# sabarim/STEm-Seg

Measured on AMD Instinct MI355X. Metric: clips/sec (T=8, 480p) embed+cluster, higher is better.
Workload: dtype f16x3: fp32 emulated from 2 fp16 terms per operand (22-bit operand significands; fp32 has 24), power-of-two operand scaling, 3 fp16 MFMA products per fp32 product, fp32 accumulate; |activation| >= 2.6e5 -> non-finite, flagged on the device, clip re-run in bf16x6

## Files before the change

stem-seg_amd/csrc/bottleneck_fused.hip:

```cpp
#include "common.h"
#include "split_operand.h"

namespace stemseg {

typedef float f32x16 __attribute__((ext_vector_type(16)));
typedef _Float16 f16x8 __attribute__((ext_vector_type(8)));
typedef unsigned int u32x4 __attribute__((ext_vector_type(4)));

struct FusedTailParams {
    const unsigned int* x16;
    const char* w3;
    const float* b3;
    const float* res;
    float* y;
    const char* w1;
    const float* b1;
    float* z;
    int64_t z_cs, z_ts, z_ys;
    int dec_H, dec_W;
    int V;
};

constexpr SplitLayout FT_WL = SplitLayout(1, STEMSEG_PRECISION_F16X3);
static_assert(FT_WL.CK == 32 && FT_WL.G == 2 && FT_WL.NPL == 2, "the fused tail walks 32-channel chunks of two k-groups, two planes");

template <int MID_, int CT_, int P_>
struct FusedTailCfg {
    static constexpr int MID = MID_, CT = CT_, COUT = 4 * MID_;
    static constexpr int P = P_, NW = P_ / 32, NTHREADS = 64 * NW;
    static constexpr int NC3 = MID / 32;
    static constexpr int NCT = COUT / CT;
    static constexpr int MI3 = CT / 32, MI1 = MID / 32;
    static constexpr int NH = 2 * MI3;
    static constexpr int X_BYTES = 2 * 4 * P * 16;
    static constexpr int W3_BYTES = 8 * CT * 16;
    static constexpr int W1_HALF = 4 * MID * 16;
    static constexpr int LDS_BYTES = 2 * X_BYTES + 2 * W3_BYTES + 2 * W1_HALF;
    static constexpr int NQ = P / 64;
    static constexpr int X_PIECES = X_BYTES / 1024, W3_PIECES = W3_BYTES / 1024, W1_PIECES = W1_HALF / 1024;
    static_assert(NC3 == FT_WL.chunks(MID) && W3_BYTES == FT_WL.slab_bytes(CT, 32) && W1_HALF * FT_WL.G == FT_WL.slab_bytes(MID, 32), "tile byte sizes follow the packed-weight layout");
    static_assert(P % 64 == 0 && MID % 32 == 0 && CT % 32 == 0 && COUT % CT == 0, "tile shapes");
    static_assert(LDS_BYTES <= (P <= 128 ? 80 : 160) * 1024, "LDS: two 128-position workgroups, or one 256-position workgroup, per CU");
    static_assert(W3_BYTES % 1024 == 0 && W1_HALF % 1024 == 0 && X_PIECES % NW == 0, "whole DMA pieces");
    static_assert(MI1 * 16 + MI3 * 16 <= 176, "accumulators must leave room for fragments at 256 registers");
};

template <class C>
__global__ __launch_bounds__(C::NTHREADS, 2) void fused_tail_kernel(const FusedTailParams p) {
#pragma clang fp contract(off)
    __shared__ __attribute__((aligned(1024))) char smem[C::LDS_BYTES];
    char* const xbuf = smem;
    char* const w3buf = smem + 2 * C::X_BYTES;
    char* const w1buf = smem + 2 * C::X_BYTES + 2 * C::W3_BYTES;

    const int tid = threadIdx.x, lane = tid & 63;
    const int wave = __builtin_amdgcn_readfirstlane(tid >> 6);
    const int half = lane >> 5, l31 = lane & 31;
    const int pos0 = blockIdx.x * C::P;
    const int pos = pos0 + wave * 32 + l31;
    const bool pos_ok = pos < p.V;
    const int pos_c = min(pos, p.V - 1);
    const int64_t V = p.V;
    const unsigned int lane_off = (unsigned int)(((int64_t)(4 * half) * V + pos_c) * 4);
    auto opaque = [](unsigned int v) __attribute__((always_inline)) { asm volatile("" : "+v"(v)); return v; };

    typedef const __attribute__((address_space(1))) void* gptr_t;
    typedef __attribute__((address_space(3))) void* lptr_t;
    const float* inv3 = reinterpret_cast<const float*>(p.w3 + FT_WL.inv_offset(C::COUT, C::MID));
    const float* inv1 = reinterpret_cast<const float*>(p.w1 + FT_WL.inv_offset(C::MID, C::COUT));

    const int xpos = min(pos0 + lane, p.V - 1);
    auto dma_x = [&](const int c, const int buf) __attribute__((always_inline)) {
#pragma unroll
        for (int k = 0; k < C::X_PIECES / C::NW; ++k) {
            const int idx = wave * (C::X_PIECES / C::NW) + k, q = idx % C::NQ, o = (idx / C::NQ) & 3, pl = idx / (4 * C::NQ);
            const unsigned int xp = (unsigned int)min((int)opaque((unsigned int)xpos) + q * 64, p.V - 1);
            const char* src = reinterpret_cast<const char*>(p.x16) + ((int64_t)(pl * (C::MID / 8) + 4 * c + o)) * V * 16 + (size_t)(xp * 16u);
            __builtin_amdgcn_global_load_lds((gptr_t)src, (lptr_t)(xbuf + buf * C::X_BYTES + ((pl * 4 + o) * C::P + q * 64) * 16), 16, 0, 0);
        }
    };
    auto dma_w3 = [&](const int j, const int c, const int buf) __attribute__((always_inline)) {
        constexpr int PER_ROW = C::CT * 16 / 1024;
#pragma unroll
        for (int k = 0; k < (C::W3_PIECES + C::NW - 1) / C::NW; ++k) {
            const int idx = wave + k * C::NW;
            if (idx < C::W3_PIECES) {
                const int row = idx / PER_ROW, part = idx % PER_ROW;
                const char* src = p.w3 + ((int64_t)c * 8 + row) * (C::COUT * 16) + (int64_t)j * (C::CT * 16) + part * 1024 + (size_t)(opaque((unsigned int)lane) * 16u);
                __builtin_amdgcn_global_load_lds((gptr_t)src, (lptr_t)(w3buf + buf * C::W3_BYTES + idx * 1024), 16, 0, 0);
            }
        }
    };
    auto dma_w1 = [&](const int j, const int h, const int buf) __attribute__((always_inline)) {
#pragma unroll
        for (int k = 0; k < (C::W1_PIECES + C::NW - 1) / C::NW; ++k) {
            const int idx = wave + k * C::NW;
            if (idx < C::W1_PIECES) {
                const char* src = p.w1 + ((int64_t)j * C::NH + h) * C::W1_HALF + (int64_t)idx * 1024 + (size_t)(opaque((unsigned int)lane) * 16u);
                __builtin_amdgcn_global_load_lds((gptr_t)src, (lptr_t)(w1buf + buf * C::W1_HALF + idx * 1024), 16, 0, 0);
            }
        }
    };
    auto dma_tab = [&](const int j, const int buf) __attribute__((always_inline)) {
        static_assert(2 * (C::CT / 4) <= 64 && 2 * C::CT * 4 <= C::W3_BYTES, "the table is one DMA piece");
        if (wave == 0 && lane < 2 * (C::CT / 4)) {
            const unsigned int l = opaque((unsigned int)lane);
            const float* src = (l < C::CT / 4 ? inv3 : p.b3 - C::CT) + (int64_t)j * C::CT + (size_t)(l * 4u);
            __builtin_amdgcn_global_load_lds((gptr_t)src, (lptr_t)(w3buf + buf * C::W3_BYTES), 16, 0, 0);
        }
    };
    auto dma_tail_tab = [&]() __attribute__((always_inline)) {
        constexpr int PIECES = (2 * C::MID + 255) / 256;
        if (wave < PIECES) {
            const unsigned int f0 = (unsigned int)wave * 256u + opaque((unsigned int)lane) * 4u;
            if (f0 < 2u * C::MID) {
                const float* src = (f0 < (unsigned int)C::MID ? inv1 : p.b1 - C::MID) + (size_t)f0;
                __builtin_amdgcn_global_load_lds((gptr_t)src, (lptr_t)(xbuf + wave * 1024), 16, 0, 0);
            }
        }
    };
    auto stage_sync = [&]() __attribute__((always_inline)) {
        __builtin_amdgcn_s_waitcnt(0x0f70);
        __syncthreads();
    };
    auto load_identity = [&](const int co_first, float (&rres)[16]) __attribute__((always_inline)) {
#pragma unroll
        for (int r = 0; r < 16; ++r)
            rres[r] = *reinterpret_cast<const float*>(reinterpret_cast<const char*>(p.res + (int64_t)(co_first + (r & 3) + 8 * (r >> 2)) * V) + (size_t)lane_off);
    };

    f32x16 acc1[C::MI1];
#pragma unroll
    for (int m = 0; m < C::MI1; ++m)
#pragma unroll
        for (int r = 0; r < 16; ++r) acc1[m][r] = 0.f;

    const f16x8 k2048 = {(_Float16)(1.0f / F16X3_LO_SCALE), (_Float16)(1.0f / F16X3_LO_SCALE), (_Float16)(1.0f / F16X3_LO_SCALE), (_Float16)(1.0f / F16X3_LO_SCALE),
                         (_Float16)(1.0f / F16X3_LO_SCALE), (_Float16)(1.0f / F16X3_LO_SCALE), (_Float16)(1.0f / F16X3_LO_SCALE), (_Float16)(1.0f / F16X3_LO_SCALE)};

    auto mma3 = [&](f32x16& acc, const f16x8 a_hi, const f16x8 a_lo, const f16x8 b_hi, const f16x8 b_lo) __attribute__((always_inline)) {
        const f16x8 a_his = a_hi * k2048;
        acc = __builtin_amdgcn_mfma_f32_32x32x16_f16(a_lo, b_hi, acc, 0, 0, 0);
        acc = __builtin_amdgcn_mfma_f32_32x32x16_f16(a_his, b_lo, acc, 0, 0, 0);
        acc = __builtin_amdgcn_mfma_f32_32x32x16_f16(a_hi, b_hi, acc, 0, 0, 0);
    };

    dma_x(0, 0);
    dma_w3(0, 0, 0);
    stage_sync();
    int sb = 0;
#pragma unroll 1
    for (int j = 0; j < C::NCT; ++j) {
        f32x16 acc3[C::MI3];
#pragma unroll
        for (int m = 0; m < C::MI3; ++m)
#pragma unroll
            for (int r = 0; r < 16; ++r) acc3[m][r] = 0.f;
        const int co_j = j * C::CT;
        float rres[16];
#pragma unroll 1
        for (int c = 0; c < C::NC3; ++c) {
            if (c + 1 < C::NC3) { dma_x(c + 1, sb ^ 1); dma_w3(j, c + 1, sb ^ 1); }
            else { dma_w1(j, 0, 0); dma_tab(j, sb ^ 1); load_identity(co_j, rres); }
            const char* xb = xbuf + sb * C::X_BYTES + (half * C::P + wave * 32 + l31) * 16;
            const char* wb = w3buf + sb * C::W3_BYTES + (half * C::CT + l31) * 16;
            constexpr int NS = 2 * C::MI3;
            f16x8 b_hi[2], b_lo[2], a_hi[2], a_lo[2];
            auto ld_b = [&](const int g, const int k) __attribute__((always_inline)) {
                b_hi[k] = *reinterpret_cast<const f16x8*>(xb + ((0 * 4 + 2 * g) * C::P) * 16);
                b_lo[k] = *reinterpret_cast<const f16x8*>(xb + ((1 * 4 + 2 * g) * C::P) * 16);
            };
            auto ld_a = [&](const int st, const int k) __attribute__((always_inline)) {
                const int g = st / C::MI3, m = st % C::MI3;
                a_hi[k] = *reinterpret_cast<const f16x8*>(wb + (((g * 2 + 0) * 2) * C::CT + m * 32) * 16);
                a_lo[k] = *reinterpret_cast<const f16x8*>(wb + (((g * 2 + 1) * 2) * C::CT + m * 32) * 16);
            };
            ld_b(0, 0);
            ld_b(1, 1);
            ld_a(0, 0);
#pragma unroll
            for (int st = 0; st < NS; ++st) {
                if (st + 1 < NS) ld_a(st + 1, (st + 1) & 1);
                __builtin_amdgcn_sched_barrier(0);
                mma3(acc3[st % C::MI3], a_hi[st & 1], a_lo[st & 1], b_hi[st / C::MI3], b_lo[st / C::MI3]);
                __builtin_amdgcn_sched_barrier(0);
            }
            stage_sync();
            sb ^= 1;
        }
        f16x8 b_hi[2], b_lo[2];
#pragma unroll
        for (int h = 0; h < C::NH; ++h) {
            const int m = h >> 1, g = h & 1;
            if (g == 0) {
                const int co_m = co_j + m * 32;
                unsigned int hw[8], lw[8];
                const float* tab = reinterpret_cast<const float*>(w3buf + sb * C::W3_BYTES);
                __builtin_amdgcn_sched_barrier(0);
#pragma unroll
                for (int q = 0; q < 4; ++q) {
                    const int co4 = co_m + 8 * q + 4 * half;
                    const float4 sc = *reinterpret_cast<const float4*>(tab + (co4 - co_j));
                    const float4 bv = *reinterpret_cast<const float4*>(tab + C::CT + (co4 - co_j));
                    float v0 = __fmul_rn(acc3[m][4 * q + 0], sc.x), v1 = __fmul_rn(acc3[m][4 * q + 1], sc.y), v2 = __fmul_rn(acc3[m][4 * q + 2], sc.z),
                          v3 = __fmul_rn(acc3[m][4 * q + 3], sc.w);
                    v0 = relu_keep_nan(__fadd_rn(__fadd_rn(v0, bv.x), rres[4 * q + 0]));
                    v1 = relu_keep_nan(__fadd_rn(__fadd_rn(v1, bv.y), rres[4 * q + 1]));
                    v2 = relu_keep_nan(__fadd_rn(__fadd_rn(v2, bv.z), rres[4 * q + 2]));
                    v3 = relu_keep_nan(__fadd_rn(__fadd_rn(v3, bv.w), rres[4 * q + 3]));
                    if (pos_ok) {
                        char* yo = reinterpret_cast<char*>(p.y + (int64_t)(co_m + 8 * q) * V);
                        *reinterpret_cast<float*>(yo + (size_t)lane_off) = v0;
                        *reinterpret_cast<float*>(yo + V * 4 + (size_t)lane_off) = v1;
                        *reinterpret_cast<float*>(yo + V * 8 + (size_t)lane_off) = v2;
                        *reinterpret_cast<float*>(yo + V * 12 + (size_t)lane_off) = v3;
                    }
                    split_pair_f16(v0, v1, hw[2 * q], lw[2 * q]);
                    split_pair_f16(v2, v3, hw[2 * q + 1], lw[2 * q + 1]);
                }
                __builtin_amdgcn_sched_barrier(0);
#pragma unroll
                for (int gg = 0; gg < 2; ++gg) {
                    unsigned int xh[2], yh[2], xl[2], yl[2];
#pragma unroll
                    for (int i = 0; i < 2; ++i) {
                        auto sh = __builtin_amdgcn_permlane32_swap(hw[4 * gg + i], hw[4 * gg + 2 + i], false, false);
                        xh[i] = sh[0]; yh[i] = sh[1];
                        auto sl = __builtin_amdgcn_permlane32_swap(lw[4 * gg + i], lw[4 * gg + 2 + i], false, false);
                        xl[i] = sl[0]; yl[i] = sl[1];
                    }
                    const u32x4 bh = {xh[0], xh[1], yh[0], yh[1]}, bl = {xl[0], xl[1], yl[0], yl[1]};
                    b_hi[gg] = __builtin_bit_cast(f16x8, bh);
                    b_lo[gg] = __builtin_bit_cast(f16x8, bl);
                }
            } else if (m + 1 < C::MI3) {
                load_identity(co_j + (m + 1) * 32, rres);
            }
            __builtin_amdgcn_sched_barrier(0);
            if (h + 1 < C::NH) dma_w1(j, h + 1, (h + 1) & 1);
            else if (j + 1 < C::NCT) { dma_x(0, sb); dma_w3(j + 1, 0, sb); }
            else dma_tail_tab();
            const char* w1b = w1buf + (h & 1) * C::W1_HALF + (half * C::MID + l31) * 16;
            f16x8 a_hi[2], a_lo[2];
            auto ld_a1 = [&](const int m1, const int k) __attribute__((always_inline)) {
                a_hi[k] = *reinterpret_cast<const f16x8*>(w1b + ((0 * 2) * C::MID + m1 * 32) * 16);
                a_lo[k] = *reinterpret_cast<const f16x8*>(w1b + ((1 * 2) * C::MID + m1 * 32) * 16);
            };
            ld_a1(0, 0);
#pragma unroll
            for (int m1 = 0; m1 < C::MI1; ++m1) {
                if (m1 + 1 < C::MI1) ld_a1(m1 + 1, (m1 + 1) & 1);
                __builtin_amdgcn_sched_barrier(0);
                mma3(acc1[m1], a_hi[m1 & 1], a_lo[m1 & 1], b_hi[g], b_lo[g]);
                __builtin_amdgcn_sched_barrier(0);
            }
            stage_sync();
        }
    }
    if (pos_ok) {
        const int hwp = p.dec_H * p.dec_W;
        const int t2 = pos / hwp, r2 = pos - t2 * hwp, y2 = r2 / p.dec_W, x2 = r2 - y2 * p.dec_W;
        const unsigned int z_off = (unsigned int)(((int64_t)(4 * half) * p.z_cs + (int64_t)t2 * p.z_ts + (int64_t)y2 * p.z_ys + x2) * 4);
#pragma unroll
        for (int m1 = 0; m1 < C::MI1; ++m1)
#pragma unroll
            for (int q = 0; q < 4; ++q) {
                const int co4 = m1 * 32 + 8 * q + 4 * half;
                const float4 sc = *reinterpret_cast<const float4*>(reinterpret_cast<const float*>(xbuf) + co4);
                const float4 bv = *reinterpret_cast<const float4*>(reinterpret_cast<const float*>(xbuf) + C::MID + co4);
                char* zo = reinterpret_cast<char*>(p.z + (int64_t)(m1 * 32 + 8 * q) * p.z_cs);
                *reinterpret_cast<float*>(zo + (size_t)z_off) = relu_keep_nan(__fadd_rn(__fmul_rn(acc1[m1][4 * q + 0], sc.x), bv.x));
                *reinterpret_cast<float*>(zo + p.z_cs * 4 + (size_t)z_off) = relu_keep_nan(__fadd_rn(__fmul_rn(acc1[m1][4 * q + 1], sc.y), bv.y));
                *reinterpret_cast<float*>(zo + p.z_cs * 8 + (size_t)z_off) = relu_keep_nan(__fadd_rn(__fmul_rn(acc1[m1][4 * q + 2], sc.z), bv.z));
                *reinterpret_cast<float*>(zo + p.z_cs * 12 + (size_t)z_off) = relu_keep_nan(__fadd_rn(__fmul_rn(acc1[m1][4 * q + 3], sc.w), bv.w));
            }
    }
}


typedef float f32x4 __attribute__((ext_vector_type(4)));

template <int MID_>
struct FusedTail16Cfg {
    static constexpr int MID = MID_, COUT = 4 * MID_, CT = 128;
    static constexpr int NW = 8, NTHREADS = 512, P = 16 * NW;
    static constexpr int NC3 = MID / 32, NCT = COUT / CT;
    static constexpr int NT3 = CT / 16, NT1 = MID / 16;
    static constexpr int SC = 2;
    static constexpr int NS = NC3 / SC, NU = CT / 32;
    static constexpr int W3_CHUNK = 8 * CT * 16;
    static constexpr int W3_BYTES = SC * W3_CHUNK;
    static constexpr int W1_BYTES = 8 * MID * 16;
    static constexpr int TAB_BYTES = 2 * CT * 4;
    static constexpr int LDS_BYTES = 2 * W3_BYTES + 2 * W1_BYTES + 2 * TAB_BYTES;
    static_assert(NC3 % SC == 0 && W3_BYTES % (1024 * NW) == 0 && W1_BYTES % (1024 * NW) == 0 && TAB_BYTES == 1024, "whole DMA pieces per wave");
    static_assert(W3_CHUNK == FT_WL.slab_bytes(CT, FT_WL.CK) && W1_BYTES == FT_WL.slab_bytes(MID, FT_WL.CK), "tile byte sizes follow the packed-weight layout");
    static_assert(LDS_BYTES <= 160 * 1024 && 2 * MID * 4 <= W3_BYTES, "LDS");
};

template <class C>
__global__ __launch_bounds__(C::NTHREADS, 2) void fused_tail16_kernel(const FusedTailParams p) {
#pragma clang fp contract(off)
    __shared__ __attribute__((aligned(1024))) char smem[C::LDS_BYTES];
    char* const w3buf = smem;
    char* const w1buf = smem + 2 * C::W3_BYTES;
    char* const tabbuf = smem + 2 * C::W3_BYTES + 2 * C::W1_BYTES;

    const int tid = threadIdx.x, lane = tid & 63;
    const int wave = __builtin_amdgcn_readfirstlane(tid >> 6);
    const int n = lane & 15, kb = lane >> 4;
    const int pos = blockIdx.x * C::P + wave * 16 + n;
    const bool pos_ok = pos < p.V;
    const int pos_c = min(pos, p.V - 1);
    const int64_t V = p.V;
    const unsigned int lane_off = (unsigned int)(((int64_t)(4 * kb) * V + pos_c) * 4);
    auto opaque = [](unsigned int v) __attribute__((always_inline)) { asm volatile("" : "+v"(v)); return v; };
    typedef const __attribute__((address_space(1))) void* gptr_t;
    typedef __attribute__((address_space(3))) void* lptr_t;
    const float* inv3 = reinterpret_cast<const float*>(p.w3 + FT_WL.inv_offset(C::COUT, C::MID));
    const float* inv1 = reinterpret_cast<const float*>(p.w1 + FT_WL.inv_offset(C::MID, C::COUT));

    auto dma_w3 = [&](const int j, const int st, const int buf) __attribute__((always_inline)) {
        constexpr int PER_ROW = C::CT * 16 / 1024, PER_CHUNK = C::W3_CHUNK / 1024;
#pragma unroll
        for (int k = 0; k < C::W3_BYTES / 1024 / C::NW; ++k) {
            const int idx = wave + k * C::NW, sc = idx / PER_CHUNK, r = idx % PER_CHUNK, row = r / PER_ROW, part = r % PER_ROW;
            const char* src = p.w3 + ((int64_t)(st * C::SC + sc) * 8 + row) * (C::COUT * 16) + (int64_t)j * (C::CT * 16) + part * 1024 + (size_t)(opaque((unsigned int)lane) * 16u);
            __builtin_amdgcn_global_load_lds((gptr_t)src, (lptr_t)(w3buf + buf * C::W3_BYTES + idx * 1024), 16, 0, 0);
        }
    };
    auto dma_w1 = [&](const int cc, const int buf) __attribute__((always_inline)) {
#pragma unroll
        for (int k = 0; k < C::W1_BYTES / 1024 / C::NW; ++k) {
            const int idx = wave + k * C::NW;
            const char* src = p.w1 + (int64_t)cc * C::W1_BYTES + (int64_t)idx * 1024 + (size_t)(opaque((unsigned int)lane) * 16u);
            __builtin_amdgcn_global_load_lds((gptr_t)src, (lptr_t)(w1buf + buf * C::W1_BYTES + idx * 1024), 16, 0, 0);
        }
    };
    auto dma_tab = [&](const int j) __attribute__((always_inline)) {
        if (wave == 0) {
            const unsigned int l = opaque((unsigned int)lane);
            const float* src = (l < 32 ? inv3 : p.b3 - C::CT) + (int64_t)j * C::CT + (size_t)(l * 4u);
            __builtin_amdgcn_global_load_lds((gptr_t)src, (lptr_t)(tabbuf + (j & 1) * C::TAB_BYTES), 16, 0, 0);
        }
    };
    auto dma_tail_tab = [&]() __attribute__((always_inline)) {
        constexpr int PIECES = (2 * C::MID + 255) / 256;
        if (wave < PIECES) {
            const unsigned int f0 = (unsigned int)wave * 256u + opaque((unsigned int)lane) * 4u;
            if (f0 < 2u * C::MID) {
                const float* src = (f0 < (unsigned int)C::MID ? inv1 : p.b1 - C::MID) + (size_t)f0;
                __builtin_amdgcn_global_load_lds((gptr_t)src, (lptr_t)(w3buf + wave * 1024), 16, 0, 0);
            }
        }
    };
    auto stage_sync = [&]() __attribute__((always_inline)) {
        __builtin_amdgcn_s_waitcnt(0x0f70);
        __syncthreads();
    };
    auto load_identity = [&](const int co_first, float (&rres)[8]) __attribute__((always_inline)) {
#pragma unroll
        for (int i = 0; i < 8; ++i)
            rres[i] = *reinterpret_cast<const float*>(reinterpret_cast<const char*>(p.res + (int64_t)(co_first + 16 * (i >> 2) + (i & 3)) * V) + (size_t)lane_off);
    };
    const f16x8 k2048 = {(_Float16)(1.0f / F16X3_LO_SCALE), (_Float16)(1.0f / F16X3_LO_SCALE), (_Float16)(1.0f / F16X3_LO_SCALE), (_Float16)(1.0f / F16X3_LO_SCALE),
                         (_Float16)(1.0f / F16X3_LO_SCALE), (_Float16)(1.0f / F16X3_LO_SCALE), (_Float16)(1.0f / F16X3_LO_SCALE), (_Float16)(1.0f / F16X3_LO_SCALE)};
    auto mma3x2 = [&](f32x4& c0, f32x4& c1, const f16x8 a0_hi, const f16x8 a0_lo, const f16x8 a1_hi, const f16x8 a1_lo, const f16x8 b_hi, const f16x8 b_lo)
        __attribute__((always_inline)) {
        const f16x8 a0_his = a0_hi * k2048, a1_his = a1_hi * k2048;
        c0 = __builtin_amdgcn_mfma_f32_16x16x32_f16(a0_lo, b_hi, c0, 0, 0, 0);
        c1 = __builtin_amdgcn_mfma_f32_16x16x32_f16(a1_lo, b_hi, c1, 0, 0, 0);
        c0 = __builtin_amdgcn_mfma_f32_16x16x32_f16(a0_his, b_lo, c0, 0, 0, 0);
        c1 = __builtin_amdgcn_mfma_f32_16x16x32_f16(a1_his, b_lo, c1, 0, 0, 0);
        c0 = __builtin_amdgcn_mfma_f32_16x16x32_f16(a0_hi, b_hi, c0, 0, 0, 0);
        c1 = __builtin_amdgcn_mfma_f32_16x16x32_f16(a1_hi, b_hi, c1, 0, 0, 0);
    };

    dma_w3(0, 0, 0);
    f16x8 xh[C::NC3], xl[C::NC3];
    {
        const char* xs = reinterpret_cast<const char*>(p.x16) + (size_t)((unsigned int)pos_c * 16u);
#pragma unroll
        for (int s = 0; s < C::NC3; ++s) {
            xh[s] = *reinterpret_cast<const f16x8*>(xs + ((int64_t)(4 * s + kb)) * V * 16);
            xl[s] = *reinterpret_cast<const f16x8*>(xs + ((int64_t)(C::MID / 8 + 4 * s + kb)) * V * 16);
        }
    }
    f32x4 acc1[C::NT1];
#pragma unroll
    for (int m = 0; m < C::NT1; ++m) acc1[m] = f32x4{0.f, 0.f, 0.f, 0.f};
    stage_sync();
    int sb = 0, eb = 0;
#pragma unroll 1
    for (int j = 0; j < C::NCT; ++j) {
        f32x4 acc3[C::NT3];
#pragma unroll
        for (int t = 0; t < C::NT3; ++t) acc3[t] = f32x4{0.f, 0.f, 0.f, 0.f};
        const int co_j = j * C::CT;
        float rres[8];
#pragma unroll
        for (int st = 0; st < C::NS; ++st) {
            if (st + 1 < C::NS) dma_w3(j, st + 1, sb ^ 1);
            else { dma_w1(j * C::NU, eb); dma_tab(j); load_identity(co_j, rres); }
            const char* wb = w3buf + sb * C::W3_BYTES + (((kb >> 1) * 2 * 2 + (kb & 1)) * C::CT + n) * 16;
            constexpr int NSTEP = C::SC * C::NT3 / 2;
            f16x8 a_hi[2][2], a_lo[2][2];
            auto ld_a = [&](const int i, const int k) __attribute__((always_inline)) {
                const int sc = (2 * i) / C::NT3, t = (2 * i) % C::NT3;
#pragma unroll
                for (int e = 0; e < 2; ++e) {
                    a_hi[k][e] = *reinterpret_cast<const f16x8*>(wb + sc * C::W3_CHUNK + (0 * 2 * C::CT + (t + e) * 16) * 16);
                    a_lo[k][e] = *reinterpret_cast<const f16x8*>(wb + sc * C::W3_CHUNK + (1 * 2 * C::CT + (t + e) * 16) * 16);
                }
            };
            ld_a(0, 0);
#pragma unroll
            for (int i = 0; i < NSTEP; ++i) {
                if (i + 1 < NSTEP) ld_a(i + 1, (i + 1) & 1);
                __builtin_amdgcn_sched_barrier(0);
                const int t = (2 * i) % C::NT3, ch = st * C::SC + (2 * i) / C::NT3;
                mma3x2(acc3[t], acc3[t + 1], a_hi[i & 1][0], a_lo[i & 1][0], a_hi[i & 1][1], a_lo[i & 1][1], xh[ch], xl[ch]);
                __builtin_amdgcn_sched_barrier(0);
            }
            stage_sync();
            sb ^= 1;
        }
        const float* tab = reinterpret_cast<const float*>(tabbuf + (j & 1) * C::TAB_BYTES);
#pragma unroll
        for (int u = 0; u < C::NU; ++u) {
            unsigned int hw[4], lw[4];
            __builtin_amdgcn_sched_barrier(0);
#pragma unroll
            for (int tt = 0; tt < 2; ++tt) {
                const int t = 2 * u + tt, co4 = 16 * t + 4 * kb;
                const float4 sc = *reinterpret_cast<const float4*>(tab + co4);
                const float4 bv = *reinterpret_cast<const float4*>(tab + C::CT + co4);
                float v0 = __fmul_rn(acc3[t][0], sc.x), v1 = __fmul_rn(acc3[t][1], sc.y), v2 = __fmul_rn(acc3[t][2], sc.z), v3 = __fmul_rn(acc3[t][3], sc.w);
                v0 = relu_keep_nan(__fadd_rn(__fadd_rn(v0, bv.x), rres[4 * tt + 0]));
                v1 = relu_keep_nan(__fadd_rn(__fadd_rn(v1, bv.y), rres[4 * tt + 1]));
                v2 = relu_keep_nan(__fadd_rn(__fadd_rn(v2, bv.z), rres[4 * tt + 2]));
                v3 = relu_keep_nan(__fadd_rn(__fadd_rn(v3, bv.w), rres[4 * tt + 3]));
                if (pos_ok) {
                    char* yo = reinterpret_cast<char*>(p.y + (int64_t)(co_j + 16 * t) * V);
                    *reinterpret_cast<float*>(yo + (size_t)lane_off) = v0;
                    *reinterpret_cast<float*>(yo + V * 4 + (size_t)lane_off) = v1;
                    *reinterpret_cast<float*>(yo + V * 8 + (size_t)lane_off) = v2;
                    *reinterpret_cast<float*>(yo + V * 12 + (size_t)lane_off) = v3;
                }
                split_pair_f16(v0, v1, hw[2 * tt], lw[2 * tt]);
                split_pair_f16(v2, v3, hw[2 * tt + 1], lw[2 * tt + 1]);
            }
            unsigned int bw[2][4];
#pragma unroll
            for (int pl = 0; pl < 2; ++pl)
#pragma unroll
                for (int i = 0; i < 2; ++i) {
                    const unsigned int t0 = pl ? lw[i] : hw[i], t1 = pl ? lw[2 + i] : hw[2 + i];
                    auto s32 = __builtin_amdgcn_permlane32_swap(t0, t1, false, false);
                    auto s16 = __builtin_amdgcn_permlane16_swap(s32[0], s32[1], false, false);
                    bw[pl][i] = s16[0];
                    bw[pl][2 + i] = s16[1];
                }
            const u32x4 bh = {bw[0][0], bw[0][1], bw[0][2], bw[0][3]}, bl = {bw[1][0], bw[1][1], bw[1][2], bw[1][3]};
            const f16x8 b_hi = __builtin_bit_cast(f16x8, bh), b_lo = __builtin_bit_cast(f16x8, bl);
            __builtin_amdgcn_sched_barrier(0);
            if (u + 1 < C::NU) { dma_w1(j * C::NU + u + 1, eb ^ 1); load_identity(co_j + 32 * (u + 1), rres); }
            else if (j + 1 < C::NCT) dma_w3(j + 1, 0, sb);
            else dma_tail_tab();
            __builtin_amdgcn_sched_barrier(0);
            const char* w1b = w1buf + eb * C::W1_BYTES + (((kb >> 1) * 2 * 2 + (kb & 1)) * C::MID + n) * 16;
            f16x8 a_hi[1][2], a_lo[1][2];
            auto ld_a1 = [&](const int i, const int k) __attribute__((always_inline)) {
#pragma unroll
                for (int e = 0; e < 2; ++e) {
                    a_hi[k][e] = *reinterpret_cast<const f16x8*>(w1b + (0 * 2 * C::MID + (2 * i + e) * 16) * 16);
                    a_lo[k][e] = *reinterpret_cast<const f16x8*>(w1b + (1 * 2 * C::MID + (2 * i + e) * 16) * 16);
                }
            };
#pragma unroll
            for (int i = 0; i < C::NT1 / 2; ++i) {
                ld_a1(i, 0);
                __builtin_amdgcn_sched_barrier(0);
                mma3x2(acc1[2 * i], acc1[2 * i + 1], a_hi[0][0], a_lo[0][0], a_hi[0][1], a_lo[0][1], b_hi, b_lo);
                __builtin_amdgcn_sched_barrier(0);
            }
            stage_sync();
            eb ^= 1;
        }
    }
    if (pos_ok) {
        const int hwp = p.dec_H * p.dec_W;
        const int t2 = pos / hwp, r2 = pos - t2 * hwp, y2 = r2 / p.dec_W, x2 = r2 - y2 * p.dec_W;
        const unsigned int z_off = (unsigned int)(((int64_t)(4 * kb) * p.z_cs + (int64_t)t2 * p.z_ts + (int64_t)y2 * p.z_ys + x2) * 4);
        const float* ttab = reinterpret_cast<const float*>(w3buf);
#pragma unroll
        for (int m1 = 0; m1 < C::NT1; ++m1) {
            const int co4 = m1 * 16 + 4 * kb;
            const float4 sc = *reinterpret_cast<const float4*>(ttab + co4);
            const float4 bv = *reinterpret_cast<const float4*>(ttab + C::MID + co4);
            char* zo = reinterpret_cast<char*>(p.z + (int64_t)(m1 * 16) * p.z_cs);
            *reinterpret_cast<float*>(zo + (size_t)z_off) = relu_keep_nan(__fadd_rn(__fmul_rn(acc1[m1][0], sc.x), bv.x));
            *reinterpret_cast<float*>(zo + p.z_cs * 4 + (size_t)z_off) = relu_keep_nan(__fadd_rn(__fmul_rn(acc1[m1][1], sc.y), bv.y));
            *reinterpret_cast<float*>(zo + p.z_cs * 8 + (size_t)z_off) = relu_keep_nan(__fadd_rn(__fmul_rn(acc1[m1][2], sc.z), bv.z));
            *reinterpret_cast<float*>(zo + p.z_cs * 12 + (size_t)z_off) = relu_keep_nan(__fadd_rn(__fmul_rn(acc1[m1][3], sc.w), bv.w));
        }
    }
}


typedef __amdgpu_buffer_rsrc_t ft_rsrc_t;
#define FT_VMCNT_(n) __builtin_amdgcn_s_waitcnt(((n) & 15) | (((n) >> 4) << 14) | 0x0F70)
#define FT_VMCNT(n) FT_VMCNT_(n)
#define FT_SGB(mask, n) __builtin_amdgcn_sched_group_barrier(mask, n, 0)

template <int MID_, int CT_>
struct FusedTailR1Cfg {
    static constexpr int MID = MID_, CT = CT_, COUT = 4 * MID_;
    static constexpr int NW = 4, NTHREADS = 64 * NW, P = 32 * NW;
    static constexpr int NC3 = MID / 32, NG = MID / 16, NCT = COUT / CT;
    static constexpr int MI3 = CT / 32, MI1 = MID / 32;
    static constexpr int SC = 2;
    static constexpr int NS = NC3 / SC, NU = CT / 32;
    static constexpr int NX3 = SC * 2 * (MI3 / 2), NX1 = 2 * (MI1 / 2);
    static constexpr int W3_CHUNK = 8 * CT * 16, W3_BYTES = SC * W3_CHUNK;
    static constexpr int W1_BYTES = 8 * MID * 16;
    static_assert(W3_CHUNK == FT_WL.slab_bytes(CT, FT_WL.CK) && W1_BYTES == FT_WL.slab_bytes(MID, FT_WL.CK), "tile byte sizes follow the packed-weight layout");
    static constexpr int TAB_BYTES = 1024;
    static constexpr int LDS_BYTES = 2 * W3_BYTES + 2 * W1_BYTES + 2 * TAB_BYTES;
    static constexpr int W3_PIECES = W3_BYTES / 1024 / NW, W1_PIECES = W1_BYTES / 1024 / NW;
    static constexpr int SL = 8 / NX1, S0 = NX1 / 4, M_PPS = 8 / S0;
    static_assert(NC3 % SC == 0 && MI3 % 2 == 0 && MI1 % 2 == 0 && W3_BYTES % (1024 * NW) == 0 && W1_BYTES % (1024 * NW) == 0 && 2 * CT * 4 <= TAB_BYTES, "whole DMA pieces per wave");
    static_assert(LDS_BYTES <= 160 * 1024 && 2 * MID * 4 <= W3_BYTES && (NX1 == 8 || NX1 == 4) && NX3 == 8 && MI3 == 4 && NS >= 2 && NU >= 2 && NU % 2 == 0, "LDS / slice placement / identity buffer parity");
    static_assert(W3_PIECES == 8 && W1_PIECES <= 8, "the pieces of a stage are requested in its first steps");
    static_assert(NG * 8 + MI1 * 16 <= 256, "the conv3 input and conv1's accumulators are the AGPR half of the register file");
};

template <class C>
__global__ __launch_bounds__(C::NTHREADS, 1) void fused_tail_r1_kernel(const FusedTailParams p) {
#pragma clang fp contract(off)
    __shared__ __attribute__((aligned(1024))) char smem[C::LDS_BYTES];
    char* const w3buf = smem;
    char* const w1buf = smem + 2 * C::W3_BYTES;
    char* const tabbuf = smem + 2 * C::W3_BYTES + 2 * C::W1_BYTES;

    const int tid = threadIdx.x, lane = tid & 63;
    const int wave = __builtin_amdgcn_readfirstlane(tid >> 6);
    const int half = lane >> 5, l31 = lane & 31;
    const int pos = blockIdx.x * C::P + wave * 32 + l31;
    const bool pos_ok = pos < p.V;
    const int pos_c = min(pos, p.V - 1);
    const int64_t V = p.V;
    const unsigned int V4 = (unsigned int)p.V * 4u;
    const unsigned int lane_ld = (unsigned int)(4 * half) * V4 + (unsigned int)pos_c * 4u;
    const unsigned int lane_st = pos_ok ? lane_ld : 0xFFFFFF00u;
    const unsigned int tile_bytes = (unsigned int)C::CT * V4;
    typedef __attribute__((address_space(3))) void* lptr_t;
    const float* inv3 = reinterpret_cast<const float*>(p.w3 + FT_WL.inv_offset(C::COUT, C::MID));
    const float* inv1 = reinterpret_cast<const float*>(p.w1 + FT_WL.inv_offset(C::MID, C::COUT));

    const unsigned int lane16 = (unsigned int)lane * 16u;
    const unsigned int lds_w3 = (unsigned int)(uintptr_t)(lptr_t)w3buf, lds_w1 = (unsigned int)(uintptr_t)(lptr_t)w1buf;
    auto dma_piece = [&](const char* sbase, const unsigned int lds_addr) __attribute__((always_inline)) {
        asm volatile("s_mov_b32 m0, %0\n\ts_nop 0\n\tglobal_load_lds_dwordx4 %1, %2" : : "s"(lds_addr), "v"(lane16), "s"(sbase) : "memory");
    };
    auto dma_w3 = [&](const int j, const int st, const int buf, const int k) __attribute__((always_inline)) {
        constexpr int PER_ROW = C::CT * 16 / 1024, PER_CHUNK = C::W3_CHUNK / 1024;
        const int idx = wave + k * C::NW, sc = idx / PER_CHUNK, r = idx % PER_CHUNK, row = r / PER_ROW, part = r % PER_ROW;
        dma_piece(p.w3 + ((int64_t)(st * C::SC + sc) * 8 + row) * (C::COUT * 16) + (int64_t)j * (C::CT * 16) + part * 1024, lds_w3 + buf * C::W3_BYTES + idx * 1024);
    };
    auto dma_w1 = [&](const int cc, const int buf, const int k) __attribute__((always_inline)) {
        const int idx = wave + k * C::NW;
        dma_piece(p.w1 + (int64_t)cc * C::W1_BYTES + (int64_t)idx * 1024, lds_w1 + buf * C::W1_BYTES + idx * 1024);
    };
    float4 tabv = {0.f, 0.f, 0.f, 0.f};
    auto tab_fetch = [&](const int j) __attribute__((always_inline)) {
        if (wave == 0 && lane < 2 * (C::CT / 4))
            tabv = *reinterpret_cast<const float4*>((lane < C::CT / 4 ? inv3 : p.b3 - C::CT) + (int64_t)j * C::CT + lane * 4);
    };
    auto tab_store = [&](const int j) __attribute__((always_inline)) {
        if (wave == 0 && lane < 2 * (C::CT / 4)) *reinterpret_cast<float4*>(tabbuf + (j & 1) * C::TAB_BYTES + lane * 16) = tabv;
    };
    auto rsrc_of = [&](const float* base, const int jj) __attribute__((always_inline)) {
        return __builtin_amdgcn_make_buffer_rsrc(const_cast<float*>(base + (int64_t)jj * C::CT * V), 0, (int)tile_bytes, 0x00020000);
    };
    auto load_identity = [&](const int jj, const int u, float (&rr)[16]) __attribute__((always_inline)) {
        const ft_rsrc_t rs = rsrc_of(p.res, jj);
#pragma unroll
        for (int r = 0; r < 16; ++r)
            rr[r] = __builtin_bit_cast(float, __builtin_amdgcn_raw_buffer_load_b32(rs, lane_ld, (unsigned int)(32 * u + (r & 3) + 8 * (r >> 2)) * V4, 0));
    };
    const f16x8 k2048 = {(_Float16)(1.0f / F16X3_LO_SCALE), (_Float16)(1.0f / F16X3_LO_SCALE), (_Float16)(1.0f / F16X3_LO_SCALE), (_Float16)(1.0f / F16X3_LO_SCALE),
                         (_Float16)(1.0f / F16X3_LO_SCALE), (_Float16)(1.0f / F16X3_LO_SCALE), (_Float16)(1.0f / F16X3_LO_SCALE), (_Float16)(1.0f / F16X3_LO_SCALE)};
    auto mma6 = [&](f32x16& c0, f32x16& c1, const f16x8 (&a_hi)[2], const f16x8 (&a_lo)[2], const f16x8 (&a_his)[2], const f16x8 b_hi, const f16x8 b_lo)
        __attribute__((always_inline)) {
        c0 = __builtin_amdgcn_mfma_f32_32x32x16_f16(a_lo[0], b_hi, c0, 0, 0, 0);
        c1 = __builtin_amdgcn_mfma_f32_32x32x16_f16(a_lo[1], b_hi, c1, 0, 0, 0);
        c0 = __builtin_amdgcn_mfma_f32_32x32x16_f16(a_his[0], b_lo, c0, 0, 0, 0);
        c1 = __builtin_amdgcn_mfma_f32_32x32x16_f16(a_his[1], b_lo, c1, 0, 0, 0);
        c0 = __builtin_amdgcn_mfma_f32_32x32x16_f16(a_hi[0], b_hi, c0, 0, 0, 0);
        c1 = __builtin_amdgcn_mfma_f32_32x32x16_f16(a_hi[1], b_hi, c1, 0, 0, 0);
    };

#pragma unroll
    for (int k = 0; k < C::W3_PIECES; ++k) dma_w3(0, 0, 0, k);
    float rres[2][16];
    load_identity(0, 0, rres[0]);
    load_identity(0, 1, rres[1]);
    f16x8 xh[C::NG], xl[C::NG];
    {
        const char* xs = reinterpret_cast<const char*>(p.x16) + (size_t)((unsigned int)pos_c * 16u);
#pragma unroll
        for (int G = 0; G < C::NG; ++G) {
            xh[G] = *reinterpret_cast<const f16x8*>(xs + ((int64_t)(2 * G + half)) * V * 16);
            xl[G] = *reinterpret_cast<const f16x8*>(xs + ((int64_t)(C::MID / 8 + 2 * G + half)) * V * 16);
        }
    }
    f32x16 acc1[C::MI1];
#pragma unroll
    for (int m = 0; m < C::MI1; ++m)
#pragma unroll
        for (int r = 0; r < 16; ++r) acc1[m][r] = 0.f;
    FT_VMCNT(0);
    __syncthreads();
    int sb = 0, eb = 0;
#pragma unroll 1
    for (int j = 0; j < C::NCT; ++j) {
        f32x16 acc3[C::MI3];
#pragma unroll
        for (int m = 0; m < C::MI3; ++m)
#pragma unroll
            for (int r = 0; r < 16; ++r) acc3[m][r] = 0.f;
        const float* tab = reinterpret_cast<const float*>(tabbuf + (j & 1) * C::TAB_BYTES) + 4 * half;
        const ft_rsrc_t ry = rsrc_of(p.y, j);
        unsigned int hw[8], lw[8];
        f16x8 b_hi[2][2], b_lo[2][2];
        auto e_slice = [&](const int u, const int q4) __attribute__((always_inline)) {
            const int c4 = 32 * u + 8 * q4;
            const float4 sc = *reinterpret_cast<const float4*>(tab + c4);
            const float4 bv = *reinterpret_cast<const float4*>(tab + C::CT + c4);
            float (&rr)[16] = rres[u & 1];
            float v0 = __fmul_rn(acc3[u][4 * q4 + 0], sc.x), v1 = __fmul_rn(acc3[u][4 * q4 + 1], sc.y), v2 = __fmul_rn(acc3[u][4 * q4 + 2], sc.z),
                  v3 = __fmul_rn(acc3[u][4 * q4 + 3], sc.w);
            v0 = relu_keep_nan(__fadd_rn(__fadd_rn(v0, bv.x), rr[4 * q4 + 0]));
            v1 = relu_keep_nan(__fadd_rn(__fadd_rn(v1, bv.y), rr[4 * q4 + 1]));
            v2 = relu_keep_nan(__fadd_rn(__fadd_rn(v2, bv.z), rr[4 * q4 + 2]));
            v3 = relu_keep_nan(__fadd_rn(__fadd_rn(v3, bv.w), rr[4 * q4 + 3]));
            __builtin_amdgcn_raw_buffer_store_b32(__builtin_bit_cast(unsigned int, v0), ry, lane_st, (unsigned int)(c4 + 0) * V4, 0);
            __builtin_amdgcn_raw_buffer_store_b32(__builtin_bit_cast(unsigned int, v1), ry, lane_st, (unsigned int)(c4 + 1) * V4, 0);
            __builtin_amdgcn_raw_buffer_store_b32(__builtin_bit_cast(unsigned int, v2), ry, lane_st, (unsigned int)(c4 + 2) * V4, 0);
            __builtin_amdgcn_raw_buffer_store_b32(__builtin_bit_cast(unsigned int, v3), ry, lane_st, (unsigned int)(c4 + 3) * V4, 0);
            split_pair_f16(v0, v1, hw[2 * q4], lw[2 * q4]);
            split_pair_f16(v2, v3, hw[2 * q4 + 1], lw[2 * q4 + 1]);
        };
        auto e_perm = [&](const int gg, f16x8& bh, f16x8& bl) __attribute__((always_inline)) {
            unsigned int xh_[2], yh_[2], xl_[2], yl_[2];
#pragma unroll
            for (int i = 0; i < 2; ++i) {
                auto sh = __builtin_amdgcn_permlane32_swap(hw[4 * gg + i], hw[4 * gg + 2 + i], false, false);
                xh_[i] = sh[0]; yh_[i] = sh[1];
                auto sl = __builtin_amdgcn_permlane32_swap(lw[4 * gg + i], lw[4 * gg + 2 + i], false, false);
                xl_[i] = sl[0]; yl_[i] = sl[1];
            }
            const u32x4 bh4 = {xh_[0], xh_[1], yh_[0], yh_[1]}, bl4 = {xl_[0], xl_[1], yl_[0], yl_[1]};
            bh = __builtin_bit_cast(f16x8, bh4);
            bl = __builtin_bit_cast(f16x8, bl4);
        };
#pragma unroll
        for (int st = 0; st < C::NS; ++st) {
            if (st + 2 == C::NS) tab_fetch(j);
            const char* wb = w3buf + sb * C::W3_BYTES + (half * C::CT + l31) * 16;
            f16x8 a_hi[3][2], a_lo[3][2], a_his[2][2];
            auto ld3 = [&](const int s, const int k) __attribute__((always_inline)) {
                const int mp = s / (2 * C::SC), sc = (s % (2 * C::SC)) / 2, g = s % 2;
#pragma unroll
                for (int e = 0; e < 2; ++e) {
                    a_hi[k][e] = *reinterpret_cast<const f16x8*>(wb + sc * C::W3_CHUNK + (((g * 2 + 0) * 2) * C::CT + (2 * mp + e) * 32) * 16);
                    a_lo[k][e] = *reinterpret_cast<const f16x8*>(wb + sc * C::W3_CHUNK + (((g * 2 + 1) * 2) * C::CT + (2 * mp + e) * 32) * 16);
                }
            };
            ld3(0, 0);
            ld3(1, 1);
            a_his[0][0] = a_hi[0][0] * k2048;
            a_his[0][1] = a_hi[0][1] * k2048;
#pragma unroll
            for (int s = 0; s < C::NX3; ++s) {
                __builtin_amdgcn_sched_barrier(0);
                if (s < 2) {
#pragma unroll
                    for (int k = 4 * s; k < 4 * s + 4; ++k) {
                        if (st + 1 < C::NS) dma_w3(j, st + 1, sb ^ 1, k);
                        else if (k < C::W1_PIECES) dma_w1(j * C::NU, eb, k);
                    }
                }
                if (s + 2 < C::NX3) ld3(s + 2, (s + 2) % 3);
                if (s + 1 < C::NX3) {
                    a_his[(s + 1) & 1][0] = a_hi[(s + 1) % 3][0] * k2048;
                    a_his[(s + 1) & 1][1] = a_hi[(s + 1) % 3][1] * k2048;
                }
                if (st + 1 == C::NS && s >= C::NX3 / 2) e_slice(0, s - C::NX3 / 2);
                const int mp = s / (2 * C::SC), sc = (s % (2 * C::SC)) / 2, g = s % 2, G = 2 * (st * C::SC + sc) + g;
                mma6(acc3[2 * mp], acc3[2 * mp + 1], a_hi[s % 3], a_lo[s % 3], a_his[s & 1], xh[G], xl[G]);
#pragma unroll
                for (int i = 0; i < 6; ++i) {
                    FT_SGB(0x008, 1); FT_SGB(0x100, 1);
                    if (st + 1 == C::NS && s >= C::NX3 / 2) { FT_SGB(0x002, 7); FT_SGB(0x040, 1); }
                    else FT_SGB(0x002, 2);
                }
            }
            __builtin_amdgcn_sched_barrier(0);
            if (st + 1 == C::NS) FT_VMCNT(16);
            else FT_VMCNT(0);
            if (st + 2 == C::NS) tab_store(j);
            __syncthreads();
            sb ^= 1;
        }
        e_perm(0, b_hi[0][0], b_lo[0][0]);
        e_perm(1, b_hi[0][1], b_lo[0][1]);
#pragma unroll
        for (int u = 0; u < C::NU; ++u) {
            const char* w1b = w1buf + eb * C::W1_BYTES + (half * C::MID + l31) * 16;
            f16x8 a_hi[3][2], a_lo[3][2], a_his[2][2];
            auto ld1 = [&](const int s, const int k) __attribute__((always_inline)) {
                const int g = s / (C::MI1 / 2), mp = s % (C::MI1 / 2);
#pragma unroll
                for (int e = 0; e < 2; ++e) {
                    a_hi[k][e] = *reinterpret_cast<const f16x8*>(w1b + (((g * 2 + 0) * 2) * C::MID + (2 * mp + e) * 32) * 16);
                    a_lo[k][e] = *reinterpret_cast<const f16x8*>(w1b + (((g * 2 + 1) * 2) * C::MID + (2 * mp + e) * 32) * 16);
                }
            };
            ld1(0, 0);
            ld1(1, 1);
            a_his[0][0] = a_hi[0][0] * k2048;
            a_his[0][1] = a_hi[0][1] * k2048;
#pragma unroll
            for (int s = 0; s < C::NX1; ++s) {
                __builtin_amdgcn_sched_barrier(0);
                if (s < C::S0) {
#pragma unroll
                    for (int k = C::M_PPS * s; k < C::M_PPS * s + C::M_PPS; ++k) {
                        if (u + 1 < C::NU) { if (k < C::W1_PIECES) dma_w1(j * C::NU + u + 1, eb ^ 1, k); }
                        else if (j + 1 < C::NCT) dma_w3(j + 1, 0, sb, k);
                    }
                }
                if (s == C::S0) load_identity(u + 2 < C::NU ? j : min(j + 1, C::NCT - 1), (u + 2) % C::NU, rres[u & 1]);
                if (s + 2 < C::NX1) ld1(s + 2, (s + 2) % 3);
                if (s + 1 < C::NX1) {
                    a_his[(s + 1) & 1][0] = a_hi[(s + 1) % 3][0] * k2048;
                    a_his[(s + 1) & 1][1] = a_hi[(s + 1) % 3][1] * k2048;
                }
                if (u + 1 < C::NU) {
                    constexpr int SE = C::S0 + 4 / C::SL;
                    if (s >= C::S0 && s < SE) {
#pragma unroll
                        for (int q = 0; q < C::SL; ++q) e_slice(u + 1, (s - C::S0) * C::SL + q);
                    }
                    if (C::SL == 1 ? s == SE : s == SE) e_perm(0, b_hi[(u + 1) & 1][0], b_lo[(u + 1) & 1][0]);
                    if (C::SL == 1 ? s == SE + 1 : s == SE) e_perm(1, b_hi[(u + 1) & 1][1], b_lo[(u + 1) & 1][1]);
                }
                const int g = s / (C::MI1 / 2), mp = s % (C::MI1 / 2);
                mma6(acc1[2 * mp], acc1[2 * mp + 1], a_hi[s % 3], a_lo[s % 3], a_his[s & 1], b_hi[u & 1][g], b_lo[u & 1][g]);
#pragma unroll
                for (int i = 0; i < 6; ++i) { FT_SGB(0x008, 1); FT_SGB(0x100, 1); FT_SGB(0x002, 7 * C::SL); FT_SGB(0x040, C::SL); FT_SGB(0x020, 3); }
            }
            __builtin_amdgcn_sched_barrier(0);
            if (u + 1 < C::NU) FT_VMCNT(32);
            else FT_VMCNT(16);
            __syncthreads();
            eb ^= 1;
        }
    }
    static_assert(C::MID / 4 <= 64, "one lane per four channels");
    if (wave < 2 && lane < C::MID / 4)
        *reinterpret_cast<float4*>(w3buf + wave * (C::MID * 4) + lane * 16) = *reinterpret_cast<const float4*>((wave == 0 ? inv1 : p.b1) + lane * 4);
    __syncthreads();
    if (pos_ok) {
        const int hwp = p.dec_H * p.dec_W;
        const int t2 = pos / hwp, r2 = pos - t2 * hwp, y2 = r2 / p.dec_W, x2 = r2 - y2 * p.dec_W;
        const unsigned int z_off = (unsigned int)(((int64_t)(4 * half) * p.z_cs + (int64_t)t2 * p.z_ts + (int64_t)y2 * p.z_ys + x2) * 4);
        const float* ttab = reinterpret_cast<const float*>(w3buf);
#pragma unroll
        for (int m1 = 0; m1 < C::MI1; ++m1)
#pragma unroll
            for (int q = 0; q < 4; ++q) {
                const int co4 = m1 * 32 + 8 * q + 4 * half;
                const float4 sc = *reinterpret_cast<const float4*>(ttab + co4);
                const float4 bv = *reinterpret_cast<const float4*>(ttab + C::MID + co4);
                char* zo = reinterpret_cast<char*>(p.z + (int64_t)(m1 * 32 + 8 * q) * p.z_cs);
                *reinterpret_cast<float*>(zo + (size_t)z_off) = relu_keep_nan(__fadd_rn(__fmul_rn(acc1[m1][4 * q + 0], sc.x), bv.x));
                *reinterpret_cast<float*>(zo + p.z_cs * 4 + (size_t)z_off) = relu_keep_nan(__fadd_rn(__fmul_rn(acc1[m1][4 * q + 1], sc.y), bv.y));
                *reinterpret_cast<float*>(zo + p.z_cs * 8 + (size_t)z_off) = relu_keep_nan(__fadd_rn(__fmul_rn(acc1[m1][4 * q + 2], sc.z), bv.z));
                *reinterpret_cast<float*>(zo + p.z_cs * 12 + (size_t)z_off) = relu_keep_nan(__fadd_rn(__fmul_rn(acc1[m1][4 * q + 3], sc.w), bv.w));
            }
    }
}

template <class C>
static int launch_fused_r1_cfg(const FusedTailParams& p, hipStream_t s) {
    const double flops = 2.0 * 2.0 * (double)C::MID * C::COUT * (double)p.V;
    void* ev = profile_begin(19, flops, s);
    hipLaunchKernelGGL(fused_tail_r1_kernel<C>, dim3((unsigned)ceil_div(p.V, C::P)), dim3(C::NTHREADS), 0, s, p);
    profile_end(ev, s);
    SS_LAUNCH_CHECK();
    return STEMSEG_OK;
}

template <class C>
static int launch_fused16_cfg(const FusedTailParams& p, hipStream_t s) {
    const double flops = 2.0 * 2.0 * (double)C::MID * C::COUT * (double)p.V;
    void* ev = profile_begin(19, flops, s);
    hipLaunchKernelGGL(fused_tail16_kernel<C>, dim3((unsigned)ceil_div(p.V, C::P)), dim3(C::NTHREADS), 0, s, p);
    profile_end(ev, s);
    SS_LAUNCH_CHECK();
    return STEMSEG_OK;
}

template <class C>
static int launch_fused_cfg(const FusedTailParams& p, hipStream_t s) {
    const double flops = 2.0 * 2.0 * (double)C::MID * C::COUT * (double)p.V;
    void* ev = profile_begin(19, flops, s);
    hipLaunchKernelGGL(fused_tail_kernel<C>, dim3((unsigned)ceil_div(p.V, C::P)), dim3(C::NTHREADS), 0, s, p);
    profile_end(ev, s);
    SS_LAUNCH_CHECK();
    return STEMSEG_OK;
}

bool fused_tail_supported(int mid) { return mid == 64 || mid == 128 || mid == 256; }

int launch_fused_tail(int mid, const unsigned int* x16, const float* w3, const float* b3, const float* res, float* y, const float* w1, const float* b1,
                      const StemsegVolume& z, int dec_H, int dec_W, int64_t V, int form, hipStream_t s) {
    SS_CHECK_ARG(x16 && w3 && b3 && res && y && w1 && b1 && z.ptr, "fused_tail: null pointer");
    SS_CHECK_ARG(fused_tail_supported(mid), "fused_tail: mid = %d (64, 128 or 256)", mid);
    SS_CHECK_ARG(V > 0 && V <= (1ll << 27) && z.c_stride <= (1ll << 27) && dec_H > 0 && dec_W > 0 && V % ((int64_t)dec_H * dec_W) == 0, "fused_tail: V = %lld positions of %d x %d planes",
                 (long long)V, dec_H, dec_W);
    SS_CHECK_ARG(z.C == mid, "fused_tail: consumer volume has %d channels, conv1 makes %d", z.C, mid);
    SS_CHECK_ARG(reinterpret_cast<uintptr_t>(x16) % 16 == 0 && reinterpret_cast<uintptr_t>(w3) % 16 == 0 && reinterpret_cast<uintptr_t>(w1) % 16 == 0 &&
                 reinterpret_cast<uintptr_t>(b3) % 16 == 0 && reinterpret_cast<uintptr_t>(b1) % 16 == 0, "fused_tail: 16-byte aligned operands");
    FusedTailParams p;
    p.x16 = x16; p.w3 = reinterpret_cast<const char*>(w3); p.b3 = b3; p.res = res; p.y = y;
    p.w1 = reinterpret_cast<const char*>(w1); p.b1 = b1;
    p.z = z.ptr; p.z_cs = z.c_stride; p.z_ts = z.t_stride; p.z_ys = z.y_stride; p.dec_H = dec_H; p.dec_W = dec_W;
    p.V = (int)V;
    if (mid == 256) {
        const bool r1_fits = (int64_t)128 * V * 4 < (1ll << 32) - (1 << 20);
        if (form != 1 && r1_fits) return launch_fused_r1_cfg<FusedTailR1Cfg<256, 128>>(p, s);
        return launch_fused16_cfg<FusedTail16Cfg<256>>(p, s);
    }
    if (mid == 128 && form != 1 && (int64_t)128 * V * 4 < (1ll << 32) - (1 << 20)) return launch_fused_r1_cfg<FusedTailR1Cfg<128, 128>>(p, s);
    if (mid == 128) return launch_fused_cfg<FusedTailCfg<128, 128, 128>>(p, s);
    return launch_fused_cfg<FusedTailCfg<64, 128, 128>>(p, s);
}

}
```

stem-seg_amd/csrc/common.h:

```cpp
#pragma once
#include <hip/hip_runtime.h>
#include <cstdarg>
#include <cstdint>
#include <cstdio>
#include <cstring>

#include "../../include/stemseg_hip.h"

#if defined(__HIP_DEVICE_COMPILE__) && defined(__AMDGCN_WAVEFRONT_SIZE) && __AMDGCN_WAVEFRONT_SIZE != 64
#error "libstemseg_hip is written for 64-lane wavefronts (gfx950): shuffles, ballots and MFMA layouts assume it"
#endif

namespace stemseg {

void set_error(const char* fmt, ...);

#define SS_CHECK_ARG(cond, ...)                                     \
    do {                                                            \
        if (!(cond)) {                                              \
            ::stemseg::set_error(__VA_ARGS__);                      \
            return STEMSEG_E_INVALID;                               \
        }                                                           \
    } while (0)

#define SS_HIP(call)                                                                            \
    do {                                                                                        \
        hipError_t e_ = (call);                                                                 \
        if (e_ != hipSuccess) {                                                                 \
            ::stemseg::set_error("%s failed: %s (%s:%d)", #call, hipGetErrorString(e_),         \
                                 __FILE__, __LINE__);                                           \
            return STEMSEG_E_HIP;                                                               \
        }                                                                                       \
    } while (0)

#define SS_LAUNCH_CHECK() SS_HIP(hipGetLastError())

static inline hipStream_t as_stream(void* s) { return reinterpret_cast<hipStream_t>(s); }
static inline int64_t ceil_div(int64_t a, int64_t b) { return (a + b - 1) / b; }
static inline int64_t round_up(int64_t a, int64_t b) { return ceil_div(a, b) * b; }

__device__ __forceinline__ float relu_keep_nan(float v) { return v < 0.f ? 0.f : v; }
__device__ __forceinline__ float max_keep_nan(float a, float b) { return (a > b || a != a) ? a : b; }

struct PaddedGeom {
    int64_t pitch, ts, cs, total, interior;
    PaddedGeom() = default;
    PaddedGeom(int C, int T, int H, int W) {
        pitch = round_up((int64_t)W + 2, 4);
        ts = (int64_t)(H + 2) * pitch;
        cs = (int64_t)(T + 2) * ts;
        total = (int64_t)C * cs + 64;
        interior = ts + pitch + 1;
    }
};

static inline StemsegVolume make_volume(float* ptr, int64_t cs, int64_t ts, int64_t ys, int C, int T, int H, int W,
                                        int64_t limit) {
    StemsegVolume v;
    v.ptr = ptr; v.c_stride = cs; v.t_stride = ts; v.y_stride = ys; v.C = C; v.T = T; v.H = H; v.W = W; v.limit = limit;
    return v;
}
static inline StemsegVolume dense_volume(float* ptr, int C, int T, int H, int W) {
    return make_volume(ptr, (int64_t)T * H * W, (int64_t)H * W, W, C, T, H, W, (int64_t)C * T * H * W);
}
static inline StemsegVolume padded_halo_view(float* base, int C, int T, int H, int W) {
    PaddedGeom g(C, T, H, W);
    return make_volume(base, g.cs, g.ts, g.pitch, C, T + 2, H + 2, W + 2, g.total);
}
static inline StemsegVolume padded_interior_view(float* base, int C, int T, int H, int W) {
    PaddedGeom g(C, T, H, W);
    return make_volume(base + g.interior, g.cs, g.ts, g.pitch, C, T, H, W, g.total - g.interior);
}

constexpr int WS_GUARD_FLOATS = 64;
constexpr uint32_t WS_CANARY = 0x7fc5ca7au;
constexpr int WS_MAX_GUARDS = 64;
struct GuardList {
    int n = 0;
    int64_t off[WS_MAX_GUARDS];
    bool full = false;
    void push(int64_t o) { if (n < WS_MAX_GUARDS) off[n++] = o; else full = true; }
};
int launch_canary_fill(float* ws, const GuardList& g, hipStream_t s);
int canary_check(const float* ws, const GuardList& g, int32_t* n_bad_host, int64_t* first_bad_host, hipStream_t s);

void* profile_begin(int tag, double work, hipStream_t s);
void profile_end(void* handle, hipStream_t s);

struct ConvEpilogue {
    int relu = 0;
    const float* res = nullptr;
    int64_t res_cs = 0, res_ts = 0, res_ys = 0;
    int dec_H = 0, dec_W = 0;
    int precision = 0;
    int frames = 0, plan_frames = 0;
    int64_t plan_scratch_floats = 0;
    double* gn_part = nullptr;
    int gn_cpg = 0, gn_cap = 0;
    int* gn_used = nullptr;
    int nb = 1;
    int64_t in_bs = 0, out_bs = 0, gn_bs = 0;
    unsigned int* p16_out = nullptr;
    int* p16_done = nullptr;
    int zero_t_halo = 0;
};
int launch_conv3d(const StemsegVolume& in, const float* packed_w, const float* bias, const StemsegVolume& out,
                  int kt, int kh, int kw, int tile_cfg, hipStream_t s, float* splitk_scratch = nullptr, int64_t splitk_scratch_floats = 0,
                  const ConvEpilogue* epi = nullptr);
int launch_grouped_conv(const StemsegVolume& in, const void* packed_w, const float* bias, const StemsegVolume& out, int groups, int stride,
                        int relu, int precision, hipStream_t s);
bool fused_tail_supported(int mid);
int launch_fused_tail(int mid, const unsigned int* x16, const float* w3, const float* b3, const float* res, float* y, const float* w1, const float* b1,
                      const StemsegVolume& z, int dec_H, int dec_W, int64_t V, int form, hipStream_t s);
int launch_gn_stats(const float* x, int C, int64_t S, int groups, float eps, float* stats, double* scratch, hipStream_t s);
constexpr int GN_SLOT_CAP = 32768;
static inline int64_t gn_scratch_doubles(int Cout, int groups) { return (int64_t)groups * GN_SLOT_CAP * 2 > (int64_t)groups * 128 ? (int64_t)groups * GN_SLOT_CAP * 2 : (int64_t)groups * 128; }
int launch_conv3d_gn(const StemsegVolume& in, const float* packed_w, const float* bias, const StemsegVolume& out, int kt, int kh, int kw,
                     int tile_cfg, hipStream_t s, float* splitk_scratch, int64_t splitk_scratch_floats, const ConvEpilogue* epi, int groups,
                     float eps, float* stats, double* gn_scratch, int64_t stats_bs = 0);
int launch_gn_identity_stats(float* stats, int groups, hipStream_t s);
struct ClipBatch {
    int nb = 1;
    int64_t in_bs = 0, out_bs = 0, stats_bs = 0;
};
int launch_gn_finalize_slots(const double* part, int groups, int cap, int used, double group_elems, float eps, float* stats, hipStream_t s,
                             int nb = 1, int64_t part_bs = 0, int64_t stats_bs = 0);
int launch_gn_relu_pool(const float* x, int C, int T, int H, int W, int groups, const float* stats, const float* gamma,
                        const float* beta, int pool, const StemsegVolume& out, hipStream_t s, const ClipBatch& cb = ClipBatch());
int launch_upsample(const float* in, int C, int T, int H, int W, int st, int sy, int sx, const StemsegVolume& out,
                    hipStream_t s, const ClipBatch& cb = ClipBatch());
int launch_copy_to_volume(const float* in, int layout, const StemsegVolume& out, hipStream_t s);
int launch_copy_strided(const float* in, int64_t in_c_stride, int64_t in_t_stride, const StemsegVolume& out, hipStream_t s);
struct HeadSpec {
    int n_out;
    int act[STEMSEG_MAX_EMB_DIMS * 2];
    int grid_axis[STEMSEG_MAX_EMB_DIMS * 2];
};
struct HeadsGN {
    const float* stats;
    const float* gamma;
    const float* beta;
    int cpg;
    int64_t stats_bs;
};
int launch_heads(const float* x, int Cin, int T, int H, int W, const float* w, const float* bias, const HeadSpec& hs,
                 const float* gt, const float* gy, const float* gx, float* out, hipStream_t s, const ClipBatch& cb = ClipBatch(),
                 const float* add = nullptr, int64_t add_bs = 0, const HeadsGN* gn = nullptr);
int launch_level_head(const float* x, int Cin, int64_t V, const float* w, int n_out, const float* add, float* out, hipStream_t s, int nb, int64_t x_bs,
                      int64_t add_bs, int64_t out_bs);

}
```

stem-seg_amd/csrc/encoder.hip:

```cpp
#include "common.h"
#include <algorithm>
#include <cstddef>

namespace stemseg {

struct Padded2D {
    int64_t pitch, ts, cs, total, interior;
    Padded2D() = default;
    Padded2D(int C, int T, int H, int W) {
        pitch = round_up((int64_t)W + 2, 4);
        ts = (int64_t)(H + 2) * pitch;
        cs = (int64_t)T * ts;
        total = (int64_t)C * cs + 64;
        interior = pitch + 1;
    }
};
static inline StemsegVolume halo2d_view(float* base, int C, int T, int H, int W) {
    Padded2D g(C, T, H, W);
    return make_volume(base, g.cs, g.ts, g.pitch, C, T, H + 2, W + 2, g.total);
}
static inline StemsegVolume interior2d_view(float* base, int C, int T, int H, int W) {
    Padded2D g(C, T, H, W);
    return make_volume(base + g.interior, g.cs, g.ts, g.pitch, C, T, H, W, g.total - g.interior);
}
static inline StemsegVolume flat_view(float* base, int C, int64_t V) { return make_volume(base, V, 0, 0, C, 1, 1, (int)V, (int64_t)C * V); }

constexpr int ST_ROWS = 8, ST_COLS = 64, ST_PR = 2 * ST_ROWS + 5, ST_PC = 2 * ST_COLS + 5;

constexpr int SM_PW = 68, SM_ROWS_IN = 2 * ST_ROWS + 6;
constexpr int SM_PLANE = 3 * SM_ROWS_IN * SM_PW;
constexpr int SM_KSTEPS = 3 * 7 * 4;
typedef float f32x16s __attribute__((ext_vector_type(16)));
__global__ __launch_bounds__(256, 2) void stem_conv7x7_mfma_kernel(const float* __restrict__ frames, const float* __restrict__ w_tap_major,
                                                                 const float* __restrict__ bias, float* __restrict__ out, int T, int H, int W) {
    __shared__ __attribute__((aligned(16))) float lds[2 * SM_PLANE + SM_KSTEPS * 2 * 64];
    float* const planes = lds;
    float* const wl = lds + 2 * SM_PLANE;
    const int Ho = H / 2, Wo = W / 2;
    const int tiles_x = (Wo + ST_COLS - 1) / ST_COLS, tiles_y = (Ho + ST_ROWS - 1) / ST_ROWS;
    int b = blockIdx.x;
    const int tx = b % tiles_x; b /= tiles_x;
    const int ty = b % tiles_y;
    const int t = b / tiles_y;
    const int oy0 = ty * ST_ROWS, ox0 = tx * ST_COLS;
    const int iy0 = 2 * oy0 - 3, ix0 = 2 * ox0 - 3;
    for (int i = threadIdx.x; i < SM_KSTEPS * 2 * 64; i += 256) {
        const int co = i & 63, half = (i >> 6) & 1, step = i >> 7;
        const int q = step & 3, cdy = step >> 2, dx = 2 * q + half;
        wl[i] = dx < 7 ? w_tap_major[(cdy * 7 + dx) * 64 + co] : 0.f;
    }
    for (int i = threadIdx.x; i < 2 * SM_PLANE; i += 256) {
        const int par = i / SM_PLANE, r = i - par * SM_PLANE;
        const int xi = r % SM_PW, yy = (r / SM_PW) % SM_ROWS_IN, c = r / (SM_PW * SM_ROWS_IN);
        const int iy = iy0 + yy, ix = ix0 + 2 * xi + par;
        float v = 0.f;
        if (yy < ST_PR && 2 * xi + par < ST_PC && iy >= 0 && iy < H && ix >= 0 && ix < W) v = frames[(((int64_t)t * 3 + c) * H + iy) * W + ix];
        planes[i] = v;
    }
    __syncthreads();
    const int lane = threadIdx.x & 63, wave = threadIdx.x >> 6, half = lane >> 5, l31 = lane & 31;
    f32x16s acc[2][4];
#pragma unroll
    for (int mi = 0; mi < 2; ++mi)
#pragma unroll
        for (int ni = 0; ni < 4; ++ni)
#pragma unroll
            for (int r = 0; r < 16; ++r) acc[mi][ni][r] = 0.f;
    const float* a_ptr = wl + half * 64 + l31;
    const float* b_ptr[4];
#pragma unroll
    for (int ni = 0; ni < 4; ++ni) b_ptr[ni] = planes + half * SM_PLANE + (2 * (2 * wave + (ni >> 1))) * SM_PW + (ni & 1) * 32 + l31;
    auto ld = [&](const int step, float (&a)[2], float (&bv)[4]) __attribute__((always_inline)) {
        const int q = step & 3, cdy = step >> 2, c = cdy / 7, dy = cdy - 7 * c;
        const int boff = (c * SM_ROWS_IN + dy) * SM_PW + q;
#pragma unroll
        for (int mi = 0; mi < 2; ++mi) a[mi] = a_ptr[step * 128 + mi * 32];
#pragma unroll
        for (int ni = 0; ni < 4; ++ni) bv[ni] = b_ptr[ni][boff];
    };
    auto mm = [&](const float (&a)[2], const float (&bv)[4]) __attribute__((always_inline)) {
#pragma unroll
        for (int mi = 0; mi < 2; ++mi)
#pragma unroll
            for (int ni = 0; ni < 4; ++ni) acc[mi][ni] = __builtin_amdgcn_mfma_f32_32x32x2f32(a[mi], bv[ni], acc[mi][ni], 0, 0, 0);
    };
    float a0[2], b0[4], a1[2], b1[4];
    ld(0, a0, b0);
#pragma unroll
    for (int i = 0; i < SM_KSTEPS; i += 2) {
        ld(i + 1, a1, b1);
        __builtin_amdgcn_sched_barrier(0);
        mm(a0, b0);
        __builtin_amdgcn_sched_barrier(0);
        if (i + 2 < SM_KSTEPS) ld(i + 2, a0, b0);
        __builtin_amdgcn_sched_barrier(0);
        mm(a1, b1);
        __builtin_amdgcn_sched_barrier(0);
    }
    const int64_t plane = (int64_t)Ho * Wo;
#pragma unroll
    for (int ni = 0; ni < 4; ++ni) {
        const int oy = oy0 + 2 * wave + (ni >> 1), ox = ox0 + (ni & 1) * 32 + l31;
        if (oy < Ho && ox < Wo) {
#pragma unroll
            for (int mi = 0; mi < 2; ++mi)
#pragma unroll
                for (int r = 0; r < 16; ++r) {
                    const int ch = mi * 32 + (r & 3) + 8 * (r >> 2) + 4 * half;
                    out[((int64_t)ch * T + t) * plane + (int64_t)oy * Wo + ox] = relu_keep_nan(acc[mi][ni][r] + bias[ch]);
                }
        }
    }
}

__global__ __launch_bounds__(256) void stem_s2d_kernel(const float* __restrict__ frames, float* __restrict__ s2d, int T, int H, int W, int64_t ts, int pitch) {
    const int W2 = W / 2, H2 = H / 2;
    const int64_t total = (int64_t)T * 3 * H * W2;
    for (int64_t i = (int64_t)blockIdx.x * blockDim.x + threadIdx.x; i < total; i += (int64_t)gridDim.x * blockDim.x) {
        const int X = (int)(i % W2);
        int64_t r = i / W2;
        const int y = (int)(r % H);
        r /= H;
        const int c = (int)(r % 3), t = (int)(r / 3);
        const float2 v = *reinterpret_cast<const float2*>(frames + (((int64_t)t * 3 + c) * H + y) * W + 2 * X);
        const int p = y & 1, Y = y >> 1;
        (void)H2;
        float* o = s2d + ((int64_t)((p * 2 + 0) * 3 + c) * T + t) * ts + (int64_t)(Y + 2) * pitch + X + 2;
        o[0] = v.x;
        o[(int64_t)3 * T * ts] = v.y;
    }
}

__global__ __launch_bounds__(256) void maxpool3x3s2_kernel(const float* __restrict__ in, float* __restrict__ out, int64_t planes, int H, int W) {
    const int Ho = H / 2, Wo = W / 2;
    const int64_t total = planes * Ho * Wo;
    for (int64_t i = (int64_t)blockIdx.x * blockDim.x + threadIdx.x; i < total; i += (int64_t)gridDim.x * blockDim.x) {
        const int x = (int)(i % Wo);
        int64_t r = i / Wo;
        const int y = (int)(r % Ho);
        const int64_t pl = r / Ho;
        const float* p = in + pl * H * W;
        float m = -INFINITY;
#pragma unroll
        for (int dy = -1; dy <= 1; ++dy) {
            const int yy = 2 * y + dy;
            if (yy < 0 || yy >= H) continue;
#pragma unroll
            for (int dx = -1; dx <= 1; ++dx) {
                const int xx = 2 * x + dx;
                if (xx < 0 || xx >= W) continue;
                m = max_keep_nan(m, p[(int64_t)yy * W + xx]);
            }
        }
        out[i] = m;
    }
}

__global__ __launch_bounds__(256) void maxpool3x3s2_vec4_kernel(const float* __restrict__ in, float* __restrict__ out, int H, int W, unsigned n_items) {
    const int Ho = H / 2, Wo = W / 2;
    const unsigned wq = Wo / 4, idx = blockIdx.x * 256u + threadIdx.x;
    if (idx >= n_items) return;
    const unsigned row = idx / wq;
    const int j = (int)(idx - row * wq);
    const unsigned pl = row / (unsigned)Ho, y = row - pl * (unsigned)Ho;
    const float* p = in + (size_t)pl * H * W;
    float m[4] = {-INFINITY, -INFINITY, -INFINITY, -INFINITY};
#pragma unroll
    for (int dy = -1; dy <= 1; ++dy) {
        const int yy = 2 * (int)y + dy;
        if (yy < 0 || yy >= H) continue;
        const float* r = p + (size_t)yy * W + 8 * j;
        const float4 a = *reinterpret_cast<const float4*>(r), b = *reinterpret_cast<const float4*>(r + 4);
        const float left = j > 0 ? r[-1] : -INFINITY;
        m[0] = max_keep_nan(m[0], max_keep_nan(left, max_keep_nan(a.x, a.y)));
        m[1] = max_keep_nan(m[1], max_keep_nan(a.y, max_keep_nan(a.z, a.w)));
        m[2] = max_keep_nan(m[2], max_keep_nan(a.w, max_keep_nan(b.x, b.y)));
        m[3] = max_keep_nan(m[3], max_keep_nan(b.y, max_keep_nan(b.z, b.w)));
    }
    *reinterpret_cast<float4*>(out + (size_t)row * Wo + 4 * j) = make_float4(m[0], m[1], m[2], m[3]);
}
__global__ __launch_bounds__(256) void subsample2_vec4_kernel(const float* __restrict__ in, float* __restrict__ out, int H, int W, unsigned n_items) {
    const int Ho = H / 2, Wo = W / 2;
    const unsigned wq = Wo / 4, idx = blockIdx.x * 256u + threadIdx.x;
    if (idx >= n_items) return;
    const unsigned row = idx / wq;
    const int j = (int)(idx - row * wq);
    const unsigned pl = row / (unsigned)Ho, y = row - pl * (unsigned)Ho;
    const float* r = in + (size_t)pl * H * W + (size_t)(2 * y) * W + 8 * j;
    const float4 a = *reinterpret_cast<const float4*>(r), b = *reinterpret_cast<const float4*>(r + 4);
    *reinterpret_cast<float4*>(out + (size_t)row * Wo + 4 * j) = make_float4(a.x, a.z, b.x, b.z);
}

__global__ __launch_bounds__(256) void subsample2_kernel(const float* __restrict__ in, float* __restrict__ out, int64_t planes, int H, int W) {
    const int Ho = H / 2, Wo = W / 2;
    const int64_t total = planes * Ho * Wo;
    for (int64_t i = (int64_t)blockIdx.x * blockDim.x + threadIdx.x; i < total; i += (int64_t)gridDim.x * blockDim.x) {
        const int x = (int)(i % Wo);
        int64_t r = i / Wo;
        const int y = (int)(r % Ho);
        const int64_t pl = r / Ho;
        out[i] = in[pl * H * W + (int64_t)(2 * y) * W + 2 * x];
    }
}

__device__ __forceinline__ float up2_blend(const float c00, const float c01, const float c10, const float c11, const float wx, const float wy) {
    const float h0 = __fmaf_rn(1.f - wx, c00, __fmul_rn(wx, c01));
    const float h1 = __fmaf_rn(1.f - wx, c10, __fmul_rn(wx, c11));
    return __fmaf_rn(1.f - wy, h0, __fmul_rn(wy, h1));
}

__global__ __launch_bounds__(256) void upsample2x_add_kernel(float* __restrict__ fine, const float* __restrict__ coarse, int64_t planes, int H, int W,
                                                              int64_t f_ts, int64_t f_pitch, int64_t c_ts, int64_t c_pitch) {
    const int Hc = H / 2, Wc = W / 2;
    const int64_t total = planes * H * W;
    for (int64_t i = (int64_t)blockIdx.x * blockDim.x + threadIdx.x; i < total; i += (int64_t)gridDim.x * blockDim.x) {
        const int x = (int)(i % W);
        int64_t r = i / W;
        const int y = (int)(r % H);
        const int64_t pl = r / H;
        float sy = 0.5f * ((float)y + 0.5f) - 0.5f, sx = 0.5f * ((float)x + 0.5f) - 0.5f;
        sy = sy < 0.f ? 0.f : sy;
        sx = sx < 0.f ? 0.f : sx;
        const int y0 = (int)sy, x0 = (int)sx;
        const int y1 = y0 + (y0 < Hc - 1 ? 1 : 0), x1 = x0 + (x0 < Wc - 1 ? 1 : 0);
        const float wy = sy - (float)y0, wx = sx - (float)x0;
        const float* c = coarse + pl * c_ts;
        const float v = up2_blend(c[y0 * c_pitch + x0], c[y0 * c_pitch + x1], c[y1 * c_pitch + x0], c[y1 * c_pitch + x1], wx, wy);
        float* fo = fine + pl * f_ts + (int64_t)y * f_pitch + x;
        *fo = __fadd_rn(*fo, v);
    }
}

__global__ __launch_bounds__(256) void upsample2x_add_vec4_kernel(float* __restrict__ fine_halo, const float* __restrict__ coarse, int H, int W, unsigned gq,
                                                                   unsigned n_items, int64_t f_ts, int f_pitch, int64_t c_ts, int c_pitch) {
    const unsigned idx = blockIdx.x * 256u + threadIdx.x;
    if (idx >= n_items) return;
    const unsigned row = idx / gq;
    const int k = (int)(idx - row * gq);
    const unsigned pl = row / (unsigned)H;
    const int y = (int)(row - pl * (unsigned)H);
    const int Hc = H / 2, Wc = W / 2;
    float sy = 0.5f * ((float)y + 0.5f) - 0.5f;
    sy = sy < 0.f ? 0.f : sy;
    const int y0 = (int)sy, y1 = y0 + (y0 < Hc - 1 ? 1 : 0);
    const float wy = sy - (float)y0;
    const float* c0 = coarse + (int64_t)pl * c_ts + (int64_t)y0 * c_pitch;
    const float* c1 = coarse + (int64_t)pl * c_ts + (int64_t)y1 * c_pitch;
    float4* fp = reinterpret_cast<float4*>(fine_halo + (int64_t)pl * f_ts + (int64_t)(y + 1) * f_pitch + 4 * k);
    float4 f = *fp;
    float* fv = reinterpret_cast<float*>(&f);
#pragma unroll
    for (int j = 0; j < 4; ++j) {
        const int x = 4 * k - 1 + j;
        if (x < 0 || x >= W) continue;
        float sx = 0.5f * ((float)x + 0.5f) - 0.5f;
        sx = sx < 0.f ? 0.f : sx;
        const int x0 = (int)sx, x1 = x0 + (x0 < Wc - 1 ? 1 : 0);
        const float wx = sx - (float)x0;
        fv[j] = __fadd_rn(fv[j], up2_blend(c0[x0], c0[x1], c1[x0], c1[x1], wx, wy));
    }
    *fp = f;
}

__global__ __launch_bounds__(256) void upsample2x_add_vec4x2_kernel(float* __restrict__ fine_halo, const float* __restrict__ coarse, int H, int W, unsigned gq,
                                                                     unsigned n_items, int64_t f_ts, int f_pitch, int64_t c_ts, int c_pitch) {
    const unsigned idx = blockIdx.x * 256u + threadIdx.x;
    if (idx >= n_items) return;
    const int Hc = H / 2, Wc = W / 2;
    const unsigned rowp = idx / gq;
    const int k = (int)(idx - rowp * gq);
    const unsigned pl = rowp / (unsigned)(Hc + 1);
    const int m = (int)(rowp - pl * (unsigned)(Hc + 1));
    const bool row_a = m >= 1, row_b = m < Hc;
    const int y0 = m >= 1 ? m - 1 : 0, y1 = y0 + (y0 < Hc - 1 ? 1 : 0);
    const float wy_a = 0.25f, wy_b = m >= 1 ? 0.75f : 0.f;
    const float* c0 = coarse + (int64_t)pl * c_ts + (int64_t)y0 * c_pitch;
    const float* c1 = coarse + (int64_t)pl * c_ts + (int64_t)y1 * c_pitch;
    const int xa = min(max(2 * k - 1, 0), Wc - 1), xb = min(2 * k, Wc - 1), xc = min(2 * k + 1, Wc - 1);
    const float a0 = c0[xa], b0 = c0[xb], d0 = c0[xc], a1 = c1[xa], b1 = c1[xb], d1 = c1[xc];
    float* fbase = fine_halo + (int64_t)pl * f_ts + 4 * k;
    float4 fa = {0.f, 0.f, 0.f, 0.f}, fb = {0.f, 0.f, 0.f, 0.f};
    if (row_a) fa = *reinterpret_cast<const float4*>(fbase + (int64_t)(2 * m) * f_pitch);
    if (row_b) fb = *reinterpret_cast<const float4*>(fbase + (int64_t)(2 * m + 1) * f_pitch);
    float* va = reinterpret_cast<float*>(&fa);
    float* vb = reinterpret_cast<float*>(&fb);
#pragma unroll
    for (int j = 0; j < 4; ++j) {
        const int x = 4 * k - 1 + j;
        if (x < 0 || x >= W) continue;
        const bool first = j < 2 && x > 0;
        const float p0 = first ? a0 : (x == 0 ? a0 : b0), p1 = first ? b0 : d0;
        const float q0 = first ? a1 : (x == 0 ? a1 : b1), q1 = first ? b1 : d1;
        const float wx = x == 0 ? 0.f : ((x & 1) ? 0.25f : 0.75f);
        if (row_a) va[j] = __fadd_rn(va[j], up2_blend(p0, p1, q0, q1, wx, wy_a));
        if (row_b) vb[j] = __fadd_rn(vb[j], up2_blend(p0, p1, q0, q1, wx, wy_b));
    }
    if (row_a) *reinterpret_cast<float4*>(fbase + (int64_t)(2 * m) * f_pitch) = fa;
    if (row_b) *reinterpret_cast<float4*>(fbase + (int64_t)(2 * m + 1) * f_pitch) = fb;
}

__global__ __launch_bounds__(256) void upsample2x_add_dense_vec4x2_kernel(float* __restrict__ fine_halo, const float* __restrict__ fine_dense,
                                                                           const float* __restrict__ coarse, int H, int W, unsigned gq, unsigned n_items,
                                                                           int64_t f_ts, int f_pitch, int64_t c_ts, int c_pitch) {
    const unsigned idx = blockIdx.x * 256u + threadIdx.x;
    if (idx >= n_items) return;
    const int Hc = H / 2, Wc = W / 2;
    const unsigned rowp = idx / gq;
    const int k = (int)(idx - rowp * gq);
    const unsigned pl = rowp / (unsigned)(Hc + 1);
    const int m = (int)(rowp - pl * (unsigned)(Hc + 1));
    const bool row_a = m >= 1, row_b = m < Hc;
    const int y0 = m >= 1 ? m - 1 : 0, y1 = y0 + (y0 < Hc - 1 ? 1 : 0);
    const float wy_a = 0.25f, wy_b = m >= 1 ? 0.75f : 0.f;
    const float* c0 = coarse + (int64_t)pl * c_ts + (int64_t)y0 * c_pitch;
    const float* c1 = coarse + (int64_t)pl * c_ts + (int64_t)y1 * c_pitch;
    const int xa = min(max(2 * k - 1, 0), Wc - 1), xb = min(2 * k, Wc - 1), xc = min(2 * k + 1, Wc - 1);
    const float a0 = c0[xa], b0 = c0[xb], d0 = c0[xc], a1 = c1[xa], b1 = c1[xb], d1 = c1[xc];
    const float* dbase = fine_dense + (int64_t)pl * H * W;
    float va[4] = {0.f, 0.f, 0.f, 0.f}, vb[4] = {0.f, 0.f, 0.f, 0.f};
    const bool g_lo = k >= 1, g_hi = 4 * k < W;
    if (row_a) {
        const float* r = dbase + (int64_t)(2 * m - 1) * W;
        if (g_lo) va[0] = reinterpret_cast<const float4*>(r)[k - 1].w;
        if (g_hi) { const float4 q = reinterpret_cast<const float4*>(r)[k]; va[1] = q.x; va[2] = q.y; va[3] = q.z; }
    }
    if (row_b) {
        const float* r = dbase + (int64_t)(2 * m) * W;
        if (g_lo) vb[0] = reinterpret_cast<const float4*>(r)[k - 1].w;
        if (g_hi) { const float4 q = reinterpret_cast<const float4*>(r)[k]; vb[1] = q.x; vb[2] = q.y; vb[3] = q.z; }
    }
#pragma unroll
    for (int j = 0; j < 4; ++j) {
        const int x = 4 * k - 1 + j;
        if (x < 0 || x >= W) { va[j] = 0.f; vb[j] = 0.f; continue; }
        const bool first = j < 2 && x > 0;
        const float p0 = first ? a0 : (x == 0 ? a0 : b0), p1 = first ? b0 : d0;
        const float q0 = first ? a1 : (x == 0 ? a1 : b1), q1 = first ? b1 : d1;
        const float wx = x == 0 ? 0.f : ((x & 1) ? 0.25f : 0.75f);
        if (row_a) va[j] = __fadd_rn(va[j], up2_blend(p0, p1, q0, q1, wx, wy_a));
        if (row_b) vb[j] = __fadd_rn(vb[j], up2_blend(p0, p1, q0, q1, wx, wy_b));
    }
    float* fbase = fine_halo + (int64_t)pl * f_ts + 4 * k;
    if (row_a) *reinterpret_cast<float4*>(fbase + (int64_t)(2 * m) * f_pitch) = make_float4(va[0], va[1], va[2], va[3]);
    if (row_b) *reinterpret_cast<float4*>(fbase + (int64_t)(2 * m + 1) * f_pitch) = make_float4(vb[0], vb[1], vb[2], vb[3]);
}

static int grid1d(int64_t n) { return (int)std::max<int64_t>(1, std::min<int64_t>(ceil_div(n, 256), 256 * 16)); }

struct EncoderPlan {
    GuardList guards;
    int T, H, W, nblk[4], total_blocks;
    int h[4], w[4];
    int64_t V[4];
    int64_t S0, X1, A, B, Cst[4], M1[4], M2, DS, XS, L[4], FO[4], SK, SKfloats, total;
    int64_t S2D, s2d_ts, s2d_pitch;
    int groups, s3, mid[4];
    int64_t M1S[4];
    int plan_frames;
    int64_t plan_SKfloats;
};
constexpr int64_t ENC_PLAN_SK_FLOATS = 32ll << 20;

static int make_encoder_plan(const StemsegEncoderDesc* d, EncoderPlan& p) {
    SS_CHECK_ARG(d, "encoder: null descriptor");
    constexpr int32_t old_bytes = (int32_t)offsetof(StemsegEncoderDesc, conv2_groups);
    SS_CHECK_ARG(d->struct_bytes == (int32_t)sizeof(StemsegEncoderDesc) || d->struct_bytes == old_bytes,
                 "encoder: descriptor size mismatch (%d vs %d or %d): ABI skew", d->struct_bytes, (int)sizeof(StemsegEncoderDesc), (int)old_bytes);
    const bool has_arch = d->struct_bytes == (int32_t)sizeof(StemsegEncoderDesc);
    const int groups = has_arch && d->conv2_groups > 0 ? d->conv2_groups : 1;
    const int wpg = has_arch && d->width_per_group > 0 ? d->width_per_group : 64;
    SS_CHECK_ARG(!has_arch || (d->conv2_groups >= 0 && d->width_per_group >= 0 && (d->stride_in_3x3 == 0 || d->stride_in_3x3 == 1)),
                 "encoder: conv2_groups=%d width_per_group=%d stride_in_3x3=%d", d->conv2_groups, d->width_per_group, d->stride_in_3x3);
    if (groups == 1) {
        SS_CHECK_ARG(wpg == 64, "encoder: width_per_group=%d with one group (64 only)", wpg);
    } else {
        SS_CHECK_ARG((wpg == 4 || wpg == 8) && groups <= 1024 && (groups * wpg) % 32 == 0,
                     "encoder: %d groups x %d channels (width_per_group 4 or 8: 4..64 channels per group over the stages; groups x width a multiple of 32)",
                     groups, wpg);
    }
    p.groups = groups;
    p.s3 = has_arch ? d->stride_in_3x3 : 0;
    for (int i = 0; i < 4; ++i) p.mid[i] = (groups * wpg) << i;
    SS_CHECK_ARG(d->n_clips >= 1 && d->clip_frames >= 0 && d->clip_stride >= 0, "encoder: bad clip layout");
    if (d->clip_frames > 0) {
        SS_CHECK_ARG(d->clip_stride > 0 && (d->n_clips - 1) * d->clip_stride + d->clip_frames == d->T,
                     "encoder: %d windows of %d frames every %d frames do not cover T=%d", d->n_clips, d->clip_frames, d->clip_stride, d->T);
    } else {
        SS_CHECK_ARG(d->T % d->n_clips == 0, "encoder: T=%d is not n_clips=%d whole clips", d->T, d->n_clips);
    }
    SS_CHECK_ARG(d->T >= 1 && d->H >= 32 && d->W >= 32 && d->H % 32 == 0 && d->W % 32 == 0, "encoder: T=%d H=%d W=%d (H, W multiples of 32)", d->T, d->H, d->W);
    p.T = d->T; p.H = d->H; p.W = d->W;
    p.total_blocks = 0;
    for (int i = 0; i < 4; ++i) {
        SS_CHECK_ARG(d->blocks[i] >= 1 && d->blocks[i] <= 64, "encoder: blocks[%d]=%d", i, d->blocks[i]);
        p.nblk[i] = d->blocks[i];
        p.total_blocks += d->blocks[i];
        p.h[i] = d->H >> (2 + i); p.w[i] = d->W >> (2 + i);
        p.V[i] = (int64_t)d->T * p.h[i] * p.w[i];
    }
    SS_CHECK_ARG(p.total_blocks <= STEMSEG_MAX_ENCODER_BLOCKS, "encoder: more than %d bottleneck blocks", STEMSEG_MAX_ENCODER_BLOCKS);
    int64_t off = 0;
    p.guards.n = 0;
    auto take = [&](int64_t floats) {
        int64_t o = off;
        off += round_up(floats, 64);
        p.guards.push(off);
        off += WS_GUARD_FLOATS;
        return o;
    };
    p.S0 = take(64 * 4 * p.V[0]);
    p.s2d_pitch = round_up(d->W / 2 + 3, 4);
    p.s2d_ts = (int64_t)(d->H / 2 + 3) * p.s2d_pitch;
    p.S2D = take(12 * (int64_t)d->T * p.s2d_ts + 64);
    p.X1 = take(64 * p.V[0]);
    p.A = take(256 * p.V[0]);
    p.B = take(256 * p.V[0]);
    for (int i = 0; i < 4; ++i) {
        p.Cst[i] = take((int64_t)(256 << i) * p.V[i]);
        p.M1[i] = take(Padded2D(p.mid[i], p.T, p.h[i], p.w[i]).total);
    }
    p.M2 = take((int64_t)p.mid[0] * p.V[0]);
    p.DS = take(256 * p.V[0]);
    p.XS = take(256 * p.V[1]);
    for (int i = 0; i < 4; ++i) p.L[i] = take(Padded2D(256, p.T, p.h[i], p.w[i]).total);
    const bool shared_out = d->clip_frames > 0 && d->clip_stride < d->clip_frames && d->n_clips > 1;
    for (int i = 0; i < 4; ++i) p.FO[i] = shared_out ? take(256 * p.V[i]) : -1;
    for (int i = 0; i < 4; ++i) p.M1S[i] = (p.s3 && i > 0) ? take(Padded2D(p.mid[i], p.T, p.h[i - 1], p.w[i - 1]).total) : -1;
    SS_CHECK_ARG(d->plan_frames >= 0 && d->plan_frames <= 4096, "encoder: plan_frames=%d", d->plan_frames);
    p.plan_frames = d->plan_frames;
    p.plan_SKfloats = ENC_PLAN_SK_FLOATS;
    p.SKfloats = ENC_PLAN_SK_FLOATS * (d->plan_frames > 0 ? std::max<int64_t>(1, ceil_div(d->T, d->plan_frames)) : 1);
    p.SK = take(p.SKfloats);
    p.total = off;
    SS_CHECK_ARG(!p.guards.full, "encoder: the plan has more than %d workspace slices (GuardList)", WS_MAX_GUARDS);
    return STEMSEG_OK;
}

}

using namespace stemseg;

extern "C" size_t stemseg_hip_encoder_workspace_bytes(const StemsegEncoderDesc* desc) {
    EncoderPlan p;
    if (make_encoder_plan(desc, p) != STEMSEG_OK) return 0;
    return (size_t)p.total * sizeof(float);
}

extern "C" int stemseg_hip_encoder_plan_offsets(const StemsegEncoderDesc* desc, int64_t* out25) {
    EncoderPlan p;
    int rc = make_encoder_plan(desc, p);
    if (rc) return rc;
    SS_CHECK_ARG(out25, "encoder_plan_offsets: null pointer");
    int n = 0;
    out25[n++] = p.S0; out25[n++] = p.X1; out25[n++] = p.A; out25[n++] = p.B;
    for (int i = 0; i < 4; ++i) out25[n++] = p.Cst[i];
    for (int i = 0; i < 4; ++i) out25[n++] = p.M1[i];
    out25[n++] = p.M2; out25[n++] = p.DS; out25[n++] = p.XS;
    for (int i = 0; i < 4; ++i) out25[n++] = p.L[i];
    for (int i = 0; i < 4; ++i) out25[n++] = p.FO[i];
    out25[n++] = p.SK; out25[n++] = p.total;
    return STEMSEG_OK;
}

extern "C" int stemseg_hip_encoder_init_workspace(const StemsegEncoderDesc* desc, void* workspace, size_t ws_bytes, void* stream) {
    EncoderPlan p;
    int rc = make_encoder_plan(desc, p);
    if (rc) return rc;
    SS_CHECK_ARG(workspace && (reinterpret_cast<uintptr_t>(workspace) % 256 == 0), "encoder: workspace must be 256-byte aligned");
    if (ws_bytes < (size_t)p.total * sizeof(float)) {
        set_error("encoder: workspace too small (%zu < %zu bytes)", ws_bytes, (size_t)p.total * sizeof(float));
        return STEMSEG_E_WORKSPACE;
    }
    SS_HIP(hipMemsetAsync(workspace, 0, (size_t)p.total * sizeof(float), as_stream(stream)));
    return launch_canary_fill(reinterpret_cast<float*>(workspace), p.guards, as_stream(stream));
}

extern "C" int stemseg_hip_encoder_check_workspace(const StemsegEncoderDesc* desc, const void* workspace, size_t ws_bytes, int32_t* n_bad_host,
                                                   int64_t* first_bad_host, void* stream) {
    EncoderPlan p;
    int rc = make_encoder_plan(desc, p);
    if (rc) return rc;
    SS_CHECK_ARG(workspace && ws_bytes >= (size_t)p.total * sizeof(float), "encoder_check_workspace: bad workspace");
    return canary_check(reinterpret_cast<const float*>(workspace), p.guards, n_bad_host, first_bad_host, as_stream(stream));
}

extern "C" int stemseg_hip_stem_conv(const float* frames, const float* w_tap_major, const float* bias, float* out, int32_t T, int32_t H, int32_t W,
                                     void* stream) {
    SS_CHECK_ARG(frames && w_tap_major && bias && out, "stem_conv: null pointer");
    SS_CHECK_ARG(T >= 1 && H >= 2 && W >= 2 && H % 2 == 0 && W % 2 == 0, "stem_conv: T=%d H=%d W=%d (H, W even)", T, H, W);
    const int Ho = H / 2, Wo = W / 2;
    const int64_t blocks = ceil_div(Wo, ST_COLS) * ceil_div(Ho, ST_ROWS) * T;
    SS_CHECK_ARG(blocks < (1ll << 31), "stem_conv: too many tiles");
    hipLaunchKernelGGL(stem_conv7x7_mfma_kernel, dim3((unsigned)blocks), dim3(256), 0, as_stream(stream), frames, w_tap_major, bias, out, T, H, W);
    SS_LAUNCH_CHECK();
    return STEMSEG_OK;
}

extern "C" int stemseg_hip_encoder_forward(const StemsegEncoderDesc* desc, const StemsegEncoderWeights* wts, const float* frames,
                                           const StemsegVolume* out, void* workspace, size_t ws_bytes, void* stream) {
    EncoderPlan p;
    int rc = make_encoder_plan(desc, p);
    if (rc) return rc;
    SS_CHECK_ARG(wts && frames && out && workspace, "encoder_forward: null pointer");
    if (ws_bytes < (size_t)p.total * sizeof(float)) {
        set_error("encoder: workspace too small (%zu < %zu bytes)", ws_bytes, (size_t)p.total * sizeof(float));
        return STEMSEG_E_WORKSPACE;
    }
    SS_CHECK_ARG(wts->stem_w && wts->stem_b, "encoder_forward: null stem weights");
    for (int i = 0; i < 4; ++i) {
        for (int c = 0; c < desc->n_clips; ++c) {
            const StemsegVolume& o = out[4 * c + i];
            const int Tc_ = desc->clip_frames > 0 ? desc->clip_frames : p.T / desc->n_clips;
            SS_CHECK_ARG(o.ptr && o.C == desc->out_channels && o.T == Tc_ && o.H == p.h[i] && o.W == p.w[i],
                         "encoder_forward: output volume %d of clip %d must be [%d][%d][%d][%d]", i, c, desc->out_channels, Tc_, p.h[i], p.w[i]);
        }
        SS_CHECK_ARG(wts->fpn_inner_w[i] && wts->fpn_inner_b[i] && wts->fpn_layer_w[i] && wts->fpn_layer_b[i], "encoder_forward: null FPN weights %d", i);
    }
    SS_CHECK_ARG(desc->out_channels == 256, "encoder: out_channels must be 256");
    SS_CHECK_ARG(desc->precision == STEMSEG_PRECISION_F32 || desc->precision == STEMSEG_PRECISION_BF16X6 || desc->precision == STEMSEG_PRECISION_F16X3,
                 "encoder: precision must be 0 (f32), 2 (bf16x6) or 3 (f16x3)");
    const int prec = desc->precision;
    auto epi_for = [&](int frames) {
        ConvEpilogue e;
        e.precision = prec;
        if (p.plan_frames > 0) { e.frames = frames; e.plan_frames = p.plan_frames; e.plan_scratch_floats = p.plan_SKfloats; }
        return e;
    };
    hipStream_t s = as_stream(stream);
    float* ws = reinterpret_cast<float*>(workspace);
    const int T = p.T;

    {
        const int Ho = p.H / 2, Wo = p.W / 2;
        const int blocks = (int)(ceil_div(Wo, ST_COLS) * ceil_div(Ho, ST_ROWS) * T);
        void* ev = profile_begin(47, 4.0 * ((double)3 * T * p.H * p.W + 64.0 * T * Ho * Wo), s);
        if (wts->stem_w_s2d && prec == STEMSEG_PRECISION_F16X3 && p.W % 2 == 0) {
            hipLaunchKernelGGL(stem_s2d_kernel, dim3(grid1d((int64_t)T * 3 * p.H * (p.W / 2))), dim3(256), 0, s, frames, ws + p.S2D, T, p.H, p.W, p.s2d_ts, (int)p.s2d_pitch);
            SS_LAUNCH_CHECK();
            const StemsegVolume in = make_volume(ws + p.S2D, (int64_t)T * p.s2d_ts, p.s2d_ts, p.s2d_pitch, 12, T, Ho + 3, Wo + 3, 12 * (int64_t)T * p.s2d_ts + 64);
            ConvEpilogue es = epi_for(T);
            es.relu = 1;
            rc = launch_conv3d(in, wts->stem_w_s2d, wts->stem_b, dense_volume(ws + p.S0, 64, T, Ho, Wo), 1, 4, 4, 0, s, nullptr, 0, &es);
            if (rc) return rc;
        } else {
            hipLaunchKernelGGL(stem_conv7x7_mfma_kernel, dim3((unsigned)blocks), dim3(256), 0, s, frames, wts->stem_w, wts->stem_b, ws + p.S0, T, p.H, p.W);
        }
        profile_end(ev, s);
        SS_LAUNCH_CHECK();
        ev = profile_begin(48, 4.0 * 64.0 * T * ((double)Ho * Wo + (double)p.V[0] / T), s);
        const int64_t mp_items = (int64_t)64 * T * (Ho / 2) * (Wo / 8);
        if (Wo % 8 == 0 && mp_items < (1ll << 31))
            hipLaunchKernelGGL(maxpool3x3s2_vec4_kernel, dim3((unsigned)ceil_div(mp_items, 256)), dim3(256), 0, s, (const float*)(ws + p.S0), ws + p.X1, Ho,
                               Wo, (unsigned)mp_items);
        else
            hipLaunchKernelGGL(maxpool3x3s2_kernel, dim3(grid1d(64 * p.V[0])), dim3(256), 0, s, (const float*)(ws + p.S0), ws + p.X1, (int64_t)64 * T, Ho, Wo);
        profile_end(ev, s);
        SS_LAUNCH_CHECK();
    }
    float* x = ws + p.X1;
    int cin = 64, bi = 0;
    bool conv1_done = false;
    for (int st = 0; st < 4; ++st) {
        const int mid = p.mid[st], cout = 256 << st, h = p.h[st], w = p.w[st];
        const int64_t V = p.V[st];
        for (int b = 0; b < p.nblk[st]; ++b, ++bi) {
            const bool first = (b == 0), stride2 = first && st > 0;
            const bool s3 = stride2 && p.s3;
            const bool grouped = p.groups > 1 || s3;
            SS_CHECK_ARG(wts->conv1_w[bi] && wts->conv1_b[bi] && wts->conv2_w[bi] && wts->conv2_b[bi] && wts->conv3_w[bi] && wts->conv3_b[bi],
                         "encoder_forward: null weights for block %d", bi);
            SS_CHECK_ARG(!first || (wts->down_w[bi] && wts->down_b[bi]), "encoder_forward: block %d needs a projection shortcut", bi);
            float* xin = x;
            if (stride2) {
                void* ev = profile_begin(49, 4.0 * 2.0 * (double)cin * V, s);
                const int64_t ss_items = (int64_t)cin * T * h * (w / 4);
                if (w % 4 == 0 && ss_items < (1ll << 31))
                    hipLaunchKernelGGL(subsample2_vec4_kernel, dim3((unsigned)ceil_div(ss_items, 256)), dim3(256), 0, s, (const float*)x, ws + p.XS, 2 * h,
                                       2 * w, (unsigned)ss_items);
                else
                    hipLaunchKernelGGL(subsample2_kernel, dim3(grid1d((int64_t)cin * V)), dim3(256), 0, s, (const float*)x, ws + p.XS, (int64_t)cin * T, 2 * h, 2 * w);
                profile_end(ev, s);
                SS_LAUNCH_CHECK();
                xin = ws + p.XS;
            }
            float* y = (b == p.nblk[st] - 1) ? ws + p.Cst[st] : ((b & 1) ? ws + p.B : ws + p.A);
            const int h1 = s3 ? 2 * h : h, w1 = s3 ? 2 * w : w;
            float* m1 = ws + (s3 ? p.M1S[st] : p.M1[st]);
            if (!conv1_done) {
                ConvEpilogue e1 = epi_for(T);
                e1.relu = 1; e1.dec_H = h1; e1.dec_W = w1;
                rc = launch_conv3d(flat_view(s3 ? x : xin, cin, (int64_t)T * h1 * w1), wts->conv1_w[bi], wts->conv1_b[bi], interior2d_view(m1, mid, T, h1, w1), 1, 1,
                                   1, 0, s, ws + p.SK, p.SKfloats, &e1);
                if (rc) return rc;
            }
            const bool want_fuse = ((desc->fuse_tail >> st) & 1) && prec == STEMSEG_PRECISION_F16X3 && b + 1 < p.nblk[st] && !grouped && p.groups == 1 &&
                                   mid * 4 == cout && fused_tail_supported(mid) && V <= (1ll << 27) && (int64_t)T * (h + 2) * (w + 4) <= (1ll << 27);
            int p16_done = 0;
            if (grouped) {
                rc = launch_grouped_conv(halo2d_view(m1, mid, T, h1, w1), wts->conv2_w[bi], wts->conv2_b[bi], dense_volume(ws + p.M2, mid, T, h, w), p.groups,
                                         s3 ? 2 : 1, 1, prec, s);
            } else {
                ConvEpilogue e2 = epi_for(T);
                e2.relu = 1;
                if (want_fuse) { e2.p16_out = reinterpret_cast<unsigned int*>(ws + p.M2); e2.p16_done = &p16_done; }
                rc = launch_conv3d(halo2d_view(m1, mid, T, h, w), wts->conv2_w[bi], wts->conv2_b[bi], dense_volume(ws + p.M2, mid, T, h, w), 1, 3, 3, 0, s,
                                   ws + p.SK, p.SKfloats, &e2);
            }
            if (rc) return rc;
            const float* idt = xin;
            ConvEpilogue ed = epi_for(T);
            if (first) {
                rc = launch_conv3d(flat_view(xin, cin, V), wts->down_w[bi], wts->down_b[bi], flat_view(ws + p.DS, cout, V), 1, 1, 1, 0, s, ws + p.SK, p.SKfloats,
                                   &ed);
                if (rc) return rc;
                idt = ws + p.DS;
            }
            if (want_fuse && p16_done) {
                SS_CHECK_ARG(wts->conv1_w[bi + 1] && wts->conv1_b[bi + 1], "encoder_forward: null weights for block %d", bi + 1);
                rc = launch_fused_tail(mid, reinterpret_cast<const unsigned int*>(ws + p.M2), wts->conv3_w[bi], wts->conv3_b[bi], idt, y, wts->conv1_w[bi + 1],
                                       wts->conv1_b[bi + 1], interior2d_view(ws + p.M1[st], mid, T, h, w), h, w, V, (desc->fuse_tail >> 3) & 3, s);
                if (rc) return rc;
                conv1_done = true;
            } else {
                ConvEpilogue e3 = epi_for(T);
                e3.relu = 1; e3.res = idt; e3.res_cs = V; e3.res_ts = 0; e3.res_ys = 0;
                rc = launch_conv3d(flat_view(ws + p.M2, mid, V), wts->conv3_w[bi], wts->conv3_b[bi], flat_view(y, cout, V), 1, 1, 1, 0, s, ws + p.SK, p.SKfloats, &e3);
                if (rc) return rc;
                conv1_done = false;
            }
            x = y;
            cin = cout;
        }
    }
    for (int k = 3; k >= 0; --k) {
        const int h = p.h[k], w = p.w[k];
        ConvEpilogue e = epi_for(T), el = epi_for(T);
        e.dec_H = h; e.dec_W = w;
        Padded2D gf0(256, T, h, w);
        const unsigned gq0 = (unsigned)((w + 1) / 4 + 1);
        const bool lat_dense = k < 3 && h % 2 == 0 && w % 4 == 0 && p.h[k + 1] == h / 2 && p.w[k + 1] == w / 2 && gf0.pitch % 4 == 0 &&
                               (int64_t)4 * gq0 <= gf0.pitch && (int64_t)256 * T * (h / 2 + 1) * gq0 < (1ll << 32) - 256 &&
                               (reinterpret_cast<uintptr_t>(ws + p.L[k]) % 16 == 0) && gf0.ts % 4 == 0 && (reinterpret_cast<uintptr_t>(ws + p.A) % 16 == 0);
        if (lat_dense) {
            ConvEpilogue ed = epi_for(T);
            rc = launch_conv3d(flat_view(ws + p.Cst[k], 256 << k, p.V[k]), wts->fpn_inner_w[k], wts->fpn_inner_b[k], flat_view(ws + p.A, 256, p.V[k]), 1, 1, 1, 0, s,
                               ws + p.SK, p.SKfloats, &ed);
            if (rc) return rc;
            Padded2D gc0(256, T, p.h[k + 1], p.w[k + 1]);
            void* ev = profile_begin(50, 4.0 * 256.0 * (2.0 * p.V[k] + p.V[k + 1]), s);
            const int64_t items = (int64_t)256 * T * (h / 2 + 1) * gq0;
            hipLaunchKernelGGL(upsample2x_add_dense_vec4x2_kernel, dim3((unsigned)ceil_div(items, 256)), dim3(256), 0, s, ws + p.L[k], (const float*)(ws + p.A),
                               (const float*)(ws + p.L[k + 1] + gc0.interior), h, w, gq0, (unsigned)items, gf0.ts, (int)gf0.pitch, gc0.ts, (int)gc0.pitch);
            profile_end(ev, s);
            SS_LAUNCH_CHECK();
        } else {
        rc = launch_conv3d(flat_view(ws + p.Cst[k], 256 << k, p.V[k]), wts->fpn_inner_w[k], wts->fpn_inner_b[k], interior2d_view(ws + p.L[k], 256, T, h, w), 1, 1, 1, 0, s,
                           ws + p.SK, p.SKfloats, &e);
        if (rc) return rc;
        }
        if (k < 3 && !lat_dense) {
            Padded2D gf(256, T, h, w), gc(256, T, p.h[k + 1], p.w[k + 1]);
            void* ev = profile_begin(50, 4.0 * 256.0 * (2.0 * p.V[k] + p.V[k + 1]), s);
            const unsigned gq = (unsigned)((w + 1) / 4 + 1);
            const int64_t ua_items = (int64_t)256 * T * h * gq;
            const bool ua_vec = gf.pitch % 4 == 0 && (int64_t)4 * gq <= gf.pitch && ua_items < (1ll << 32) - 256 && (reinterpret_cast<uintptr_t>(ws + p.L[k]) % 16 == 0) && gf.ts % 4 == 0;
            const int64_t ua2_items = (int64_t)256 * T * (h / 2 + 1) * gq;
            if (ua_vec && h % 2 == 0 && w % 2 == 0 && p.h[k + 1] == h / 2 && p.w[k + 1] == w / 2)
                hipLaunchKernelGGL(upsample2x_add_vec4x2_kernel, dim3((unsigned)ceil_div(ua2_items, 256)), dim3(256), 0, s, ws + p.L[k],
                                   (const float*)(ws + p.L[k + 1] + gc.interior), h, w, gq, (unsigned)ua2_items, gf.ts, (int)gf.pitch, gc.ts, (int)gc.pitch);
            else if (ua_vec)
                hipLaunchKernelGGL(upsample2x_add_vec4_kernel, dim3((unsigned)ceil_div(ua_items, 256)), dim3(256), 0, s, ws + p.L[k],
                                   (const float*)(ws + p.L[k + 1] + gc.interior), h, w, gq, (unsigned)ua_items, gf.ts, (int)gf.pitch, gc.ts, (int)gc.pitch);
            else
                hipLaunchKernelGGL(upsample2x_add_kernel, dim3(grid1d(256 * p.V[k])), dim3(256), 0, s, ws + p.L[k] + gf.interior,
                                   (const float*)(ws + p.L[k + 1] + gc.interior), (int64_t)256 * T, h, w, gf.ts, gf.pitch, gc.ts, gc.pitch);
            profile_end(ev, s);
            SS_LAUNCH_CHECK();
        }
        const int Tc = desc->clip_frames > 0 ? desc->clip_frames : T / desc->n_clips;
        const int Ts = desc->clip_frames > 0 ? desc->clip_stride : Tc;
        if (p.FO[k] >= 0) {
            rc = launch_conv3d(halo2d_view(ws + p.L[k], 256, T, h, w), wts->fpn_layer_w[k], wts->fpn_layer_b[k], dense_volume(ws + p.FO[k], 256, T, h, w), 1, 3, 3,
                               0, s, ws + p.SK, p.SKfloats, &el);
            if (rc) return rc;
            for (int c = 0; c < desc->n_clips; ++c) {
                rc = launch_copy_strided(ws + p.FO[k] + (int64_t)c * Ts * h * w, (int64_t)T * h * w, (int64_t)h * w, out[4 * c + k], s);
                if (rc) return rc;
            }
            continue;
        }
        bool uniform = desc->n_clips > 1 && desc->n_clips <= 65535;
        const int64_t obs = uniform ? out[4 + k].ptr - out[k].ptr : 0;
        for (int c = 1; c < desc->n_clips && uniform; ++c) {
            const StemsegVolume &a = out[4 * c + k], &b = out[k];
            uniform = a.ptr == b.ptr + c * obs && a.c_stride == b.c_stride && a.t_stride == b.t_stride && a.y_stride == b.y_stride && a.limit == b.limit;
        }
        if (uniform && obs > 0 && obs % 4 == 0) {
            StemsegVolume in = halo2d_view(ws + p.L[k], 256, T, h, w);
            ConvEpilogue ec = epi_for(Tc);
            ec.nb = desc->n_clips;
            ec.in_bs = (int64_t)Ts * in.t_stride;
            ec.out_bs = obs;
            in.limit -= (int64_t)(desc->n_clips - 1) * ec.in_bs;
            in.T = Tc;
            rc = launch_conv3d(in, wts->fpn_layer_w[k], wts->fpn_layer_b[k], out[k], 1, 3, 3, 0, s, ws + p.SK, p.SKfloats, &ec);
            if (rc) return rc;
            continue;
        }
        for (int c = 0; c < desc->n_clips; ++c) {
            StemsegVolume in = halo2d_view(ws + p.L[k], 256, T, h, w);
            in.ptr += (int64_t)c * Ts * in.t_stride;
            in.limit -= (int64_t)c * Ts * in.t_stride;
            in.T = Tc;
            const ConvEpilogue ec = epi_for(Tc);
            rc = launch_conv3d(in, wts->fpn_layer_w[k], wts->fpn_layer_b[k], out[4 * c + k], 1, 3, 3, 0, s, ws + p.SK, p.SKfloats, &ec);
            if (rc) return rc;
        }
    }
    return STEMSEG_OK;
}
```

Measured before the change: 122.8.

## Fuse downsample shortcut 1x1 conv into the bottleneck fused-tail kernel

For the first block of stages 0 and 1, the separate downsample 1x1 conv launch is removed. The fused tail kernel now computes the shortcut projection itself: it loads the block input, splits it into fp16 hi/lo terms, runs f16x3 MFMAs against the downsample weights, and adds the result in place of the identity residual. This avoids writing and re-reading the cout-channel shortcut tensor and saves a kernel launch. In exchange it adds extra MFMA work, extra accumulator registers and more weight DMA inside the tail kernel, which may hurt occupancy or the pipeline schedule.

Result: faster. 124.7, median of 6 (+1.6%).

```diff
diff --git a/stem-seg_amd/csrc/bottleneck_fused.hip b/stem-seg_amd/csrc/bottleneck_fused.hip
--- a/stem-seg_amd/csrc/bottleneck_fused.hip
+++ b/stem-seg_amd/csrc/bottleneck_fused.hip
@@ -19,14 +19,18 @@
     int64_t z_cs, z_ts, z_ys;
     int dec_H, dec_W;
     int V;
+    const float* xs;
+    const char* wd;
+    const float* bd;
 };
 
 constexpr SplitLayout FT_WL = SplitLayout(1, STEMSEG_PRECISION_F16X3);
 static_assert(FT_WL.CK == 32 && FT_WL.G == 2 && FT_WL.NPL == 2, "the fused tail walks 32-channel chunks of two k-groups, two planes");
 
-template <int MID_, int CT_, int P_>
+template <int MID_, int CT_, int P_, int DS_ = 0>
 struct FusedTailCfg {
     static constexpr int MID = MID_, CT = CT_, COUT = 4 * MID_;
+    static constexpr int DS = DS_, NCD = DS_ / 32;
     static constexpr int P = P_, NW = P_ / 32, NTHREADS = 64 * NW;
     static constexpr int NC3 = MID / 32;
     static constexpr int NCT = COUT / CT;
@@ -42,7 +46,8 @@
     static_assert(P % 64 == 0 && MID % 32 == 0 && CT % 32 == 0 && COUT % CT == 0, "tile shapes");
     static_assert(LDS_BYTES <= (P <= 128 ? 80 : 160) * 1024, "LDS: two 128-position workgroups, or one 256-position workgroup, per CU");
     static_assert(W3_BYTES % 1024 == 0 && W1_HALF % 1024 == 0 && X_PIECES % NW == 0, "whole DMA pieces");
-    static_assert(MI1 * 16 + MI3 * 16 <= 176, "accumulators must leave room for fragments at 256 registers");
+    static_assert(MI1 * 16 + MI3 * 16 + (DS ? MI3 * 16 : 0) <= 176, "accumulators must leave room for fragments at 256 registers");
+    static_assert(DS % 32 == 0 && 2 * CT * 4 <= W1_HALF, "shortcut: whole K-chunks; its (1 / scale, bias) table waits in a w1 buffer");
 };
 
 template <class C>
@@ -79,18 +84,20 @@
             __builtin_amdgcn_global_load_lds((gptr_t)src, (lptr_t)(xbuf + buf * C::X_BYTES + ((pl * 4 + o) * C::P + q * 64) * 16), 16, 0, 0);
         }
     };
-    auto dma_w3 = [&](const int j, const int c, const int buf) __attribute__((always_inline)) {
+    auto dma_wc = [&](const char* blob, const int j, const int c, const int buf) __attribute__((always_inline)) {
         constexpr int PER_ROW = C::CT * 16 / 1024;
 #pragma unroll
         for (int k = 0; k < (C::W3_PIECES + C::NW - 1) / C::NW; ++k) {
             const int idx = wave + k * C::NW;
             if (idx < C::W3_PIECES) {
                 const int row = idx / PER_ROW, part = idx % PER_ROW;
-                const char* src = p.w3 + ((int64_t)c * 8 + row) * (C::COUT * 16) + (int64_t)j * (C::CT * 16) + part * 1024 + (size_t)(opaque((unsigned int)lane) * 16u);
+                const char* src = blob + ((int64_t)c * 8 + row) * (C::COUT * 16) + (int64_t)j * (C::CT * 16) + part * 1024 + (size_t)(opaque((unsigned int)lane) * 16u);
                 __builtin_amdgcn_global_load_lds((gptr_t)src, (lptr_t)(w3buf + buf * C::W3_BYTES + idx * 1024), 16, 0, 0);
             }
         }
     };
+    auto dma_w3 = [&](const int j, const int c, const int buf) __attribute__((always_inline)) { dma_wc(p.w3, j, c, buf); };
+    auto dma_wd = [&](const int j, const int c, const int buf) __attribute__((always_inline)) { dma_wc(p.wd, j, c, buf); };
     auto dma_w1 = [&](const int j, const int h, const int buf) __attribute__((always_inline)) {
 #pragma unroll
         for (int k = 0; k < (C::W1_PIECES + C::NW - 1) / C::NW; ++k) {
@@ -108,6 +115,23 @@
             const float* src = (l < C::CT / 4 ? inv3 : p.b3 - C::CT) + (int64_t)j * C::CT + (size_t)(l * 4u);
             __builtin_amdgcn_global_load_lds((gptr_t)src, (lptr_t)(w3buf + buf * C::W3_BYTES), 16, 0, 0);
         }
+    };
+    auto dma_dtab = [&](const int j) __attribute__((always_inline)) {
+        if (wave == 0 && lane < 2 * (C::CT / 4)) {
+            const unsigned int l = opaque((unsigned int)lane);
+            const float* invd = reinterpret_cast<const float*>(p.wd + FT_WL.inv_offset(C::COUT, C::DS));
+            const float* src = (l < C::CT / 4 ? invd : p.bd - C::CT) + (int64_t)j * C::CT + (size_t)(l * 4u);
+            __builtin_amdgcn_global_load_lds((gptr_t)src, (lptr_t)(w1buf + C::W1_HALF), 16, 0, 0);
+        }
+    };
+    constexpr int NXS = C::DS > 0 ? C::DS / 2 : 1;
+    auto load_xs = [&](float (&xr)[NXS]) __attribute__((always_inline)) {
+        const unsigned int V4 = (unsigned int)p.V * 4u;
+        const __amdgpu_buffer_rsrc_t rs = __builtin_amdgcn_make_buffer_rsrc(const_cast<float*>(p.xs), 0, (int)((unsigned int)C::DS * V4), 0x00020000);
+        const unsigned int off = (unsigned int)(8 * half) * V4 + (unsigned int)pos_c * 4u;
+#pragma unroll
+        for (int i = 0; i < C::DS / 2; ++i)
+            xr[i] = __builtin_bit_cast(float, __builtin_amdgcn_raw_buffer_load_b32(rs, off, (unsigned int)(16 * (i >> 3) + (i & 7)) * V4, 0));
     };
     auto dma_tail_tab = [&]() __attribute__((always_inline)) {
         constexpr int PIECES = (2 * C::MID + 255) / 256;
@@ -145,12 +169,73 @@
         acc = __builtin_amdgcn_mfma_f32_32x32x16_f16(a_hi, b_hi, acc, 0, 0, 0);
     };
 
-    dma_x(0, 0);
-    dma_w3(0, 0, 0);
+    constexpr bool DSV = C::DS > 0;
+    float xr[NXS];
+    if constexpr (DSV) { dma_wd(0, 0, 0); load_xs(xr); }
+    else { dma_x(0, 0); dma_w3(0, 0, 0); }
     stage_sync();
     int sb = 0;
 #pragma unroll 1
     for (int j = 0; j < C::NCT; ++j) {
+        f32x16 accd[DSV ? C::MI3 : 1];
+        if constexpr (DSV) {
+            f16x8 d_hi[2 * C::NCD], d_lo[2 * C::NCD];
+#pragma unroll
+            for (int G = 0; G < 2 * C::NCD; ++G) {
+                u32x4 hw4, lw4;
+#pragma unroll
+                for (int i = 0; i < 4; ++i) {
+                    unsigned int hwd, lwd;
+                    split_pair_f16(xr[8 * G + 2 * i], xr[8 * G + 2 * i + 1], hwd, lwd);
+                    hw4[i] = hwd; lw4[i] = lwd;
+                }
+                d_hi[G] = __builtin_bit_cast(f16x8, hw4);
+                d_lo[G] = __builtin_bit_cast(f16x8, lw4);
+            }
+#pragma unroll
+            for (int m = 0; m < C::MI3; ++m)
+#pragma unroll
+                for (int r = 0; r < 16; ++r) accd[m][r] = 0.f;
+#pragma unroll
+            for (int c = 0; c < C::NCD; ++c) {
+                if (c + 1 < C::NCD) dma_wd(j, c + 1, sb ^ 1);
+                else { dma_x(0, sb ^ 1); dma_w3(j, 0, sb ^ 1); }
+                if (c == 0) dma_dtab(j);
+                const char* wb = w3buf + sb * C::W3_BYTES + (half * C::CT + l31) * 16;
+                constexpr int NS = 2 * C::MI3;
+                f16x8 a_hi[2], a_lo[2];
+                auto ld_a = [&](const int st, const int k) __attribute__((always_inline)) {
+                    const int g = st / C::MI3, m = st % C::MI3;
+                    a_hi[k] = *reinterpret_cast<const f16x8*>(wb + (((g * 2 + 0) * 2) * C::CT + m * 32) * 16);
+                    a_lo[k] = *reinterpret_cast<const f16x8*>(wb + (((g * 2 + 1) * 2) * C::CT + m * 32) * 16);
+                };
+                ld_a(0, 0);
+#pragma unroll
+                for (int st = 0; st < NS; ++st) {
+                    if (st + 1 < NS) ld_a(st + 1, (st + 1) & 1);
+                    __builtin_amdgcn_sched_barrier(0);
+                    mma3(accd[st % C::MI3], a_hi[st & 1], a_lo[st & 1], d_hi[2 * c + st / C::MI3], d_lo[2 * c + st / C::MI3]);
+                    __builtin_amdgcn_sched_barrier(0);
+                }
+                stage_sync();
+                sb ^= 1;
+            }
+            const float* dtab = reinterpret_cast<const float*>(w1buf + C::W1_HALF);
+#pragma unroll
+            for (int m = 0; m < C::MI3; ++m)
+#pragma unroll
+                for (int q = 0; q < 4; ++q) {
+                    const float4 sc = *reinterpret_cast<const float4*>(dtab + m * 32 + 8 * q + 4 * half);
+                    const float4 bv = *reinterpret_cast<const float4*>(dtab + C::CT + m * 32 + 8 * q + 4 * half);
+                    accd[m][4 * q + 0] = __fadd_rn(__fmul_rn(accd[m][4 * q + 0], sc.x), bv.x);
+                    accd[m][4 * q + 1] = __fadd_rn(__fmul_rn(accd[m][4 * q + 1], sc.y), bv.y);
+                    accd[m][4 * q + 2] = __fadd_rn(__fmul_rn(accd[m][4 * q + 2], sc.z), bv.z);
+                    accd[m][4 * q + 3] = __fadd_rn(__fmul_rn(accd[m][4 * q + 3], sc.w), bv.w);
+                }
+#pragma unroll
+            for (int m = 0; m < C::MI3; ++m) asm volatile("" : "+v"(accd[m]));
+            __builtin_amdgcn_sched_barrier(0);
+        }
         f32x16 acc3[C::MI3];
 #pragma unroll
         for (int m = 0; m < C::MI3; ++m)
@@ -161,7 +246,7 @@
 #pragma unroll 1
         for (int c = 0; c < C::NC3; ++c) {
             if (c + 1 < C::NC3) { dma_x(c + 1, sb ^ 1); dma_w3(j, c + 1, sb ^ 1); }
-            else { dma_w1(j, 0, 0); dma_tab(j, sb ^ 1); load_identity(co_j, rres); }
+            else { dma_w1(j, 0, 0); dma_tab(j, sb ^ 1); if constexpr (!DSV) load_identity(co_j, rres); }
             const char* xb = xbuf + sb * C::X_BYTES + (half * C::P + wave * 32 + l31) * 16;
             const char* wb = w3buf + sb * C::W3_BYTES + (half * C::CT + l31) * 16;
             constexpr int NS = 2 * C::MI3;
@@ -196,6 +281,10 @@
                 const int co_m = co_j + m * 32;
                 unsigned int hw[8], lw[8];
                 const float* tab = reinterpret_cast<const float*>(w3buf + sb * C::W3_BYTES);
+                if constexpr (DSV) {
+#pragma unroll
+                    for (int r = 0; r < 16; ++r) rres[r] = accd[m][r];
+                }
                 __builtin_amdgcn_sched_barrier(0);
 #pragma unroll
                 for (int q = 0; q < 4; ++q) {
@@ -234,12 +323,14 @@
                     b_lo[gg] = __builtin_bit_cast(f16x8, bl);
                 }
             } else if (m + 1 < C::MI3) {
-                load_identity(co_j + (m + 1) * 32, rres);
+                if constexpr (!DSV) load_identity(co_j + (m + 1) * 32, rres);
             }
             __builtin_amdgcn_sched_barrier(0);
             if (h + 1 < C::NH) dma_w1(j, h + 1, (h + 1) & 1);
-            else if (j + 1 < C::NCT) { dma_x(0, sb); dma_w3(j + 1, 0, sb); }
-            else dma_tail_tab();
+            else if (j + 1 < C::NCT) {
+                if constexpr (DSV) { dma_wd(j + 1, 0, sb); load_xs(xr); }
+                else { dma_x(0, sb); dma_w3(j + 1, 0, sb); }
+            } else dma_tail_tab();
             const char* w1b = w1buf + (h & 1) * C::W1_HALF + (half * C::MID + l31) * 16;
             f16x8 a_hi[2], a_lo[2];
             auto ld_a1 = [&](const int m1, const int k) __attribute__((always_inline)) {
@@ -513,14 +604,17 @@
 #define FT_VMCNT(n) FT_VMCNT_(n)
 #define FT_SGB(mask, n) __builtin_amdgcn_sched_group_barrier(mask, n, 0)
 
-template <int MID_, int CT_>
+template <int MID_, int CT_, int DS_ = 0>
 struct FusedTailR1Cfg {
     static constexpr int MID = MID_, CT = CT_, COUT = 4 * MID_;
+    static constexpr int DS = DS_, NGD = DS_ / 16;
     static constexpr int NW = 4, NTHREADS = 64 * NW, P = 32 * NW;
     static constexpr int NC3 = MID / 32, NG = MID / 16, NCT = COUT / CT;
     static constexpr int MI3 = CT / 32, MI1 = MID / 32;
     static constexpr int SC = 2;
     static constexpr int NS = NC3 / SC, NU = CT / 32;
+    static constexpr int NSD = DS / 32 / SC;
+    static_assert(DS % (32 * SC) == 0, "shortcut: whole stages");
     static constexpr int NX3 = SC * 2 * (MI3 / 2), NX1 = 2 * (MI1 / 2);
     static constexpr int W3_CHUNK = 8 * CT * 16, W3_BYTES = SC * W3_CHUNK;
     static constexpr int W1_BYTES = 8 * MID * 16;
@@ -568,6 +662,11 @@
         const int idx = wave + k * C::NW, sc = idx / PER_CHUNK, r = idx % PER_CHUNK, row = r / PER_ROW, part = r % PER_ROW;
         dma_piece(p.w3 + ((int64_t)(st * C::SC + sc) * 8 + row) * (C::COUT * 16) + (int64_t)j * (C::CT * 16) + part * 1024, lds_w3 + buf * C::W3_BYTES + idx * 1024);
     };
+    auto dma_wd = [&](const int j, const int st, const int buf, const int k) __attribute__((always_inline)) {
+        constexpr int PER_ROW = C::CT * 16 / 1024, PER_CHUNK = C::W3_CHUNK / 1024;
+        const int idx = wave + k * C::NW, sc = idx / PER_CHUNK, r = idx % PER_CHUNK, row = r / PER_ROW, part = r % PER_ROW;
+        dma_piece(p.wd + ((int64_t)(st * C::SC + sc) * 8 + row) * (C::COUT * 16) + (int64_t)j * (C::CT * 16) + part * 1024, lds_w3 + buf * C::W3_BYTES + idx * 1024);
+    };
     auto dma_w1 = [&](const int cc, const int buf, const int k) __attribute__((always_inline)) {
         const int idx = wave + k * C::NW;
         dma_piece(p.w1 + (int64_t)cc * C::W1_BYTES + (int64_t)idx * 1024, lds_w1 + buf * C::W1_BYTES + idx * 1024);
@@ -579,6 +678,16 @@
     };
     auto tab_store = [&](const int j) __attribute__((always_inline)) {
         if (wave == 0 && lane < 2 * (C::CT / 4)) *reinterpret_cast<float4*>(tabbuf + (j & 1) * C::TAB_BYTES + lane * 16) = tabv;
+    };
+    constexpr bool DSV = C::DS > 0;
+    float4 tabdv = {0.f, 0.f, 0.f, 0.f};
+    auto tabd_fetch = [&](const int j) __attribute__((always_inline)) {
+        const float* invd = reinterpret_cast<const float*>(p.wd + FT_WL.inv_offset(C::COUT, C::DS));
+        if (wave == 0 && lane < 2 * (C::CT / 4))
+            tabdv = *reinterpret_cast<const float4*>((lane < C::CT / 4 ? invd : p.bd - C::CT) + (int64_t)j * C::CT + lane * 4);
+    };
+    auto tabd_store = [&](const int j) __attribute__((always_inline)) {
+        if (wave == 0 && lane < 2 * (C::CT / 4)) *reinterpret_cast<float4*>(tabbuf + ((j + 1) & 1) * C::TAB_BYTES + lane * 16) = tabdv;
     };
     auto rsrc_of = [&](const float* base, const int jj) __attribute__((always_inline)) {
         return __builtin_amdgcn_make_buffer_rsrc(const_cast<float*>(base + (int64_t)jj * C::CT * V), 0, (int)tile_bytes, 0x00020000);
@@ -602,10 +711,15 @@
     };
 
 #pragma unroll
-    for (int k = 0; k < C::W3_PIECES; ++k) dma_w3(0, 0, 0, k);
+    for (int k = 0; k < C::W3_PIECES; ++k) {
+        if constexpr (DSV) dma_wd(0, 0, 0, k);
+        else dma_w3(0, 0, 0, k);
+    }
     float rres[2][16];
-    load_identity(0, 0, rres[0]);
-    load_identity(0, 1, rres[1]);
+    if constexpr (!DSV) {
+        load_identity(0, 0, rres[0]);
+        load_identity(0, 1, rres[1]);
+    }
     f16x8 xh[C::NG], xl[C::NG];
     {
         const char* xs = reinterpret_cast<const char*>(p.x16) + (size_t)((unsigned int)pos_c * 16u);
@@ -613,6 +727,26 @@
         for (int G = 0; G < C::NG; ++G) {
             xh[G] = *reinterpret_cast<const f16x8*>(xs + ((int64_t)(2 * G + half)) * V * 16);
             xl[G] = *reinterpret_cast<const f16x8*>(xs + ((int64_t)(C::MID / 8 + 2 * G + half)) * V * 16);
+        }
+    }
+    f16x8 xdh[DSV ? C::NGD : 1], xdl[DSV ? C::NGD : 1];
+    if constexpr (DSV) {
+        const ft_rsrc_t rx = __builtin_amdgcn_make_buffer_rsrc(const_cast<float*>(p.xs), 0, (int)((unsigned int)C::DS * V4), 0x00020000);
+        const unsigned int lane_xs = (unsigned int)(8 * half) * V4 + (unsigned int)pos_c * 4u;
+#pragma unroll
+        for (int G = 0; G < C::NGD; ++G) {
+            float xr[8];
+#pragma unroll
+            for (int i = 0; i < 8; ++i) xr[i] = __builtin_bit_cast(float, __builtin_amdgcn_raw_buffer_load_b32(rx, lane_xs, (unsigned int)(16 * G + i) * V4, 0));
+            u32x4 hw4, lw4;
+#pragma unroll
+            for (int i = 0; i < 4; ++i) {
+                unsigned int hwd, lwd;
+                split_pair_f16(xr[2 * i], xr[2 * i + 1], hwd, lwd);
+                hw4[i] = hwd; lw4[i] = lwd;
+            }
+            xdh[G] = __builtin_bit_cast(f16x8, hw4);
+            xdl[G] = __builtin_bit_cast(f16x8, lw4);
         }
     }
     f32x16 acc1[C::MI1];
@@ -625,6 +759,71 @@
     int sb = 0, eb = 0;
 #pragma unroll 1
     for (int j = 0; j < C::NCT; ++j) {
+        f32x16 accd[DSV ? C::MI3 : 1];
+        if constexpr (DSV) {
+#pragma unroll
+            for (int m = 0; m < C::MI3; ++m)
+#pragma unroll
+                for (int r = 0; r < 16; ++r) accd[m][r] = 0.f;
+#pragma unroll
+            for (int st = 0; st < C::NSD; ++st) {
+                if (st == 0) tabd_fetch(j);
+                const char* wb = w3buf + sb * C::W3_BYTES + (half * C::CT + l31) * 16;
+                f16x8 a_hi[3][2], a_lo[3][2], a_his[2][2];
+                auto ld3 = [&](const int s, const int k) __attribute__((always_inline)) {
+                    const int mp = s / (2 * C::SC), sc = (s % (2 * C::SC)) / 2, g = s % 2;
+#pragma unroll
+                    for (int e = 0; e < 2; ++e) {
+                        a_hi[k][e] = *reinterpret_cast<const f16x8*>(wb + sc * C::W3_CHUNK + (((g * 2 + 0) * 2) * C::CT + (2 * mp + e) * 32) * 16);
+                        a_lo[k][e] = *reinterpret_cast<const f16x8*>(wb + sc * C::W3_CHUNK + (((g * 2 + 1) * 2) * C::CT + (2 * mp + e) * 32) * 16);
+                    }
+                };
+                ld3(0, 0);
+                ld3(1, 1);
+                a_his[0][0] = a_hi[0][0] * k2048;
+                a_his[0][1] = a_hi[0][1] * k2048;
+#pragma unroll
+                for (int s = 0; s < C::NX3; ++s) {
+                    __builtin_amdgcn_sched_barrier(0);
+                    if (s < 2) {
+#pragma unroll
+                        for (int k = 4 * s; k < 4 * s + 4; ++k) {
+                            if (st + 1 < C::NSD) dma_wd(j, st + 1, sb ^ 1, k);
+                            else dma_w3(j, 0, sb ^ 1, k);
+                        }
+                    }
+                    if (s + 2 < C::NX3) ld3(s + 2, (s + 2) % 3);
+                    if (s + 1 < C::NX3) {
+                        a_his[(s + 1) & 1][0] = a_hi[(s + 1) % 3][0] * k2048;
+                        a_his[(s + 1) & 1][1] = a_hi[(s + 1) % 3][1] * k2048;
+                    }
+                    const int mp = s / (2 * C::SC), sc = (s % (2 * C::SC)) / 2, g = s % 2, G = 2 * (st * C::SC + sc) + g;
+                    mma6(accd[2 * mp], accd[2 * mp + 1], a_hi[s % 3], a_lo[s % 3], a_his[s & 1], xdh[G], xdl[G]);
+#pragma unroll
+                    for (int i = 0; i < 6; ++i) { FT_SGB(0x008, 1); FT_SGB(0x100, 1); FT_SGB(0x002, 2); }
+                }
+                __builtin_amdgcn_sched_barrier(0);
+                FT_VMCNT(0);
+                if (st == 0) tabd_store(j);
+                __syncthreads();
+                sb ^= 1;
+            }
+            const float* tabd = reinterpret_cast<const float*>(tabbuf + ((j + 1) & 1) * C::TAB_BYTES) + 4 * half;
+#pragma unroll
+            for (int u = 0; u < C::MI3; ++u)
+#pragma unroll
+                for (int q4 = 0; q4 < 4; ++q4) {
+                    const float4 sc = *reinterpret_cast<const float4*>(tabd + 32 * u + 8 * q4);
+                    const float4 bv = *reinterpret_cast<const float4*>(tabd + C::CT + 32 * u + 8 * q4);
+                    accd[u][4 * q4 + 0] = __fadd_rn(__fmul_rn(accd[u][4 * q4 + 0], sc.x), bv.x);
+                    accd[u][4 * q4 + 1] = __fadd_rn(__fmul_rn(accd[u][4 * q4 + 1], sc.y), bv.y);
+                    accd[u][4 * q4 + 2] = __fadd_rn(__fmul_rn(accd[u][4 * q4 + 2], sc.z), bv.z);
+                    accd[u][4 * q4 + 3] = __fadd_rn(__fmul_rn(accd[u][4 * q4 + 3], sc.w), bv.w);
+                }
+#pragma unroll
+            for (int u = 0; u < C::MI3; ++u) asm volatile("" : "+v"(accd[u]));
+            __builtin_amdgcn_sched_barrier(0);
+        }
         f32x16 acc3[C::MI3];
 #pragma unroll
         for (int m = 0; m < C::MI3; ++m)
@@ -638,13 +837,15 @@
             const int c4 = 32 * u + 8 * q4;
             const float4 sc = *reinterpret_cast<const float4*>(tab + c4);
             const float4 bv = *reinterpret_cast<const float4*>(tab + C::CT + c4);
-            float (&rr)[16] = rres[u & 1];
+            float rr[4];
+#pragma unroll
+            for (int i = 0; i < 4; ++i) rr[i] = DSV ? accd[DSV ? u : 0][4 * q4 + i] : rres[u & 1][4 * q4 + i];
             float v0 = __fmul_rn(acc3[u][4 * q4 + 0], sc.x), v1 = __fmul_rn(acc3[u][4 * q4 + 1], sc.y), v2 = __fmul_rn(acc3[u][4 * q4 + 2], sc.z),
                   v3 = __fmul_rn(acc3[u][4 * q4 + 3], sc.w);
-            v0 = relu_keep_nan(__fadd_rn(__fadd_rn(v0, bv.x), rr[4 * q4 + 0]));
-            v1 = relu_keep_nan(__fadd_rn(__fadd_rn(v1, bv.y), rr[4 * q4 + 1]));
-            v2 = relu_keep_nan(__fadd_rn(__fadd_rn(v2, bv.z), rr[4 * q4 + 2]));
-            v3 = relu_keep_nan(__fadd_rn(__fadd_rn(v3, bv.w), rr[4 * q4 + 3]));
+            v0 = relu_keep_nan(__fadd_rn(__fadd_rn(v0, bv.x), rr[0]));
+            v1 = relu_keep_nan(__fadd_rn(__fadd_rn(v1, bv.y), rr[1]));
+            v2 = relu_keep_nan(__fadd_rn(__fadd_rn(v2, bv.z), rr[2]));
+            v3 = relu_keep_nan(__fadd_rn(__fadd_rn(v3, bv.w), rr[3]));
             __builtin_amdgcn_raw_buffer_store_b32(__builtin_bit_cast(unsigned int, v0), ry, lane_st, (unsigned int)(c4 + 0) * V4, 0);
             __builtin_amdgcn_raw_buffer_store_b32(__builtin_bit_cast(unsigned int, v1), ry, lane_st, (unsigned int)(c4 + 1) * V4, 0);
             __builtin_amdgcn_raw_buffer_store_b32(__builtin_bit_cast(unsigned int, v2), ry, lane_st, (unsigned int)(c4 + 2) * V4, 0);
@@ -739,10 +940,10 @@
 #pragma unroll
                     for (int k = C::M_PPS * s; k < C::M_PPS * s + C::M_PPS; ++k) {
                         if (u + 1 < C::NU) { if (k < C::W1_PIECES) dma_w1(j * C::NU + u + 1, eb ^ 1, k); }
-                        else if (j + 1 < C::NCT) dma_w3(j + 1, 0, sb, k);
+                        else if (j + 1 < C::NCT) { if constexpr (DSV) dma_wd(j + 1, 0, sb, k); else dma_w3(j + 1, 0, sb, k); }
                     }
                 }
-                if (s == C::S0) load_identity(u + 2 < C::NU ? j : min(j + 1, C::NCT - 1), (u + 2) % C::NU, rres[u & 1]);
+                if (!DSV && s == C::S0) load_identity(u + 2 < C::NU ? j : min(j + 1, C::NCT - 1), (u + 2) % C::NU, rres[u & 1]);
                 if (s + 2 < C::NX1) ld1(s + 2, (s + 2) % 3);
                 if (s + 1 < C::NX1) {
                     a_his[(s + 1) & 1][0] = a_hi[(s + 1) % 3][0] * k2048;
@@ -763,8 +964,8 @@
                 for (int i = 0; i < 6; ++i) { FT_SGB(0x008, 1); FT_SGB(0x100, 1); FT_SGB(0x002, 7 * C::SL); FT_SGB(0x040, C::SL); FT_SGB(0x020, 3); }
             }
             __builtin_amdgcn_sched_barrier(0);
-            if (u + 1 < C::NU) FT_VMCNT(32);
-            else FT_VMCNT(16);
+            if (u + 1 < C::NU) FT_VMCNT(DSV ? 16 : 32);
+            else FT_VMCNT(DSV ? 0 : 16);
             __syncthreads();
             eb ^= 1;
         }
@@ -826,9 +1027,16 @@
 
 bool fused_tail_supported(int mid) { return mid == 64 || mid == 128 || mid == 256; }
 
+bool fused_shortcut_supported(int mid, int cin, int64_t V) {
+    return ((mid == 64 && cin == 64) || (mid == 128 && cin == 256)) && (int64_t)cin * V * 4 < (1ll << 32) - (1 << 20) && (int64_t)128 * V * 4 < (1ll << 32) - (1 << 20);
+}
+
 int launch_fused_tail(int mid, const unsigned int* x16, const float* w3, const float* b3, const float* res, float* y, const float* w1, const float* b1,
-                      const StemsegVolume& z, int dec_H, int dec_W, int64_t V, int form, hipStream_t s) {
-    SS_CHECK_ARG(x16 && w3 && b3 && res && y && w1 && b1 && z.ptr, "fused_tail: null pointer");
+                      const StemsegVolume& z, int dec_H, int dec_W, int64_t V, int form, hipStream_t s, const float* ds_x, int ds_cin, const float* ds_w,
+                      const float* ds_b) {
+    SS_CHECK_ARG(x16 && w3 && b3 && y && w1 && b1 && z.ptr, "fused_tail: null pointer");
+    SS_CHECK_ARG(ds_x ? (!res && ds_w && ds_b && fused_shortcut_supported(mid, ds_cin, V) && reinterpret_cast<uintptr_t>(ds_w) % 16 == 0 && reinterpret_cast<uintptr_t>(ds_b) % 16 == 0)
+                      : res != nullptr, "fused_tail: identity map, or a shortcut (mid %d, %d input channels) this library has a kernel for", mid, ds_cin);
     SS_CHECK_ARG(fused_tail_supported(mid), "fused_tail: mid = %d (64, 128 or 256)", mid);
     SS_CHECK_ARG(V > 0 && V <= (1ll << 27) && z.c_stride <= (1ll << 27) && dec_H > 0 && dec_W > 0 && V % ((int64_t)dec_H * dec_W) == 0, "fused_tail: V = %lld positions of %d x %d planes",
                  (long long)V, dec_H, dec_W);
@@ -840,6 +1048,9 @@
     p.w1 = reinterpret_cast<const char*>(w1); p.b1 = b1;
     p.z = z.ptr; p.z_cs = z.c_stride; p.z_ts = z.t_stride; p.z_ys = z.y_stride; p.dec_H = dec_H; p.dec_W = dec_W;
     p.V = (int)V;
+    p.xs = ds_x; p.wd = reinterpret_cast<const char*>(ds_w); p.bd = ds_b;
+    if (ds_x && mid == 128) return launch_fused_r1_cfg<FusedTailR1Cfg<128, 128, 256>>(p, s);
+    if (ds_x) return launch_fused_cfg<FusedTailCfg<64, 128, 128, 64>>(p, s);
     if (mid == 256) {
         const bool r1_fits = (int64_t)128 * V * 4 < (1ll << 32) - (1 << 20);
         if (form != 1 && r1_fits) return launch_fused_r1_cfg<FusedTailR1Cfg<256, 128>>(p, s);
diff --git a/stem-seg_amd/csrc/common.h b/stem-seg_amd/csrc/common.h
--- a/stem-seg_amd/csrc/common.h
+++ b/stem-seg_amd/csrc/common.h
@@ -111,7 +111,9 @@
                         int relu, int precision, hipStream_t s);
 bool fused_tail_supported(int mid);
 int launch_fused_tail(int mid, const unsigned int* x16, const float* w3, const float* b3, const float* res, float* y, const float* w1, const float* b1,
-                      const StemsegVolume& z, int dec_H, int dec_W, int64_t V, int form, hipStream_t s);
+                      const StemsegVolume& z, int dec_H, int dec_W, int64_t V, int form, hipStream_t s, const float* ds_x = nullptr, int ds_cin = 0,
+                      const float* ds_w = nullptr, const float* ds_b = nullptr);
+bool fused_shortcut_supported(int mid, int cin, int64_t V);
 int launch_gn_stats(const float* x, int C, int64_t S, int groups, float eps, float* stats, double* scratch, hipStream_t s);
 constexpr int GN_SLOT_CAP = 32768;
 static inline int64_t gn_scratch_doubles(int Cout, int groups) { return (int64_t)groups * GN_SLOT_CAP * 2 > (int64_t)groups * 128 ? (int64_t)groups * GN_SLOT_CAP * 2 : (int64_t)groups * 128; }
diff --git a/stem-seg_amd/csrc/encoder.hip b/stem-seg_amd/csrc/encoder.hip
--- a/stem-seg_amd/csrc/encoder.hip
+++ b/stem-seg_amd/csrc/encoder.hip
@@ -609,7 +609,9 @@
             if (rc) return rc;
             const float* idt = xin;
             ConvEpilogue ed = epi_for(T);
-            if (first) {
+            const bool ds_in_tail = first && want_fuse && p16_done && !(desc->fuse_tail & 32) && st < 2 && !(st == 1 && ((desc->fuse_tail >> 3) & 3) == 1) &&
+                                    fused_shortcut_supported(mid, cin, V);
+            if (first && !ds_in_tail) {
                 rc = launch_conv3d(flat_view(xin, cin, V), wts->down_w[bi], wts->down_b[bi], flat_view(ws + p.DS, cout, V), 1, 1, 1, 0, s, ws + p.SK, p.SKfloats,
                                    &ed);
                 if (rc) return rc;
@@ -617,8 +619,9 @@
             }
             if (want_fuse && p16_done) {
                 SS_CHECK_ARG(wts->conv1_w[bi + 1] && wts->conv1_b[bi + 1], "encoder_forward: null weights for block %d", bi + 1);
-                rc = launch_fused_tail(mid, reinterpret_cast<const unsigned int*>(ws + p.M2), wts->conv3_w[bi], wts->conv3_b[bi], idt, y, wts->conv1_w[bi + 1],
-                                       wts->conv1_b[bi + 1], interior2d_view(ws + p.M1[st], mid, T, h, w), h, w, V, (desc->fuse_tail >> 3) & 3, s);
+                rc = launch_fused_tail(mid, reinterpret_cast<const unsigned int*>(ws + p.M2), wts->conv3_w[bi], wts->conv3_b[bi], ds_in_tail ? nullptr : idt, y,
+                                       wts->conv1_w[bi + 1], wts->conv1_b[bi + 1], interior2d_view(ws + p.M1[st], mid, T, h, w), h, w, V, (desc->fuse_tail >> 3) & 3, s,
+                                       ds_in_tail ? xin : nullptr, cin, ds_in_tail ? wts->down_w[bi] : nullptr, ds_in_tail ? wts->down_b[bi] : nullptr);
                 if (rc) return rc;
                 conv1_done = true;
             } else {
```
